# oiwn/toy-heaan-ckks

Measured on AMD Instinct MI355X. Metric: RNS-NTT poly-muls/sec (N=2^16, 16 primes) at 1/2/4/8 GPUs; % HBM roofline, higher is better.
Workload: dtype u32

## Files before the change

toy-heaan-ckks_amd/csrc/rnt_mfma.hip:

```cpp
#include <hip/hip_runtime.h>

#include <vector>

#include "rnt_internal.hpp"
#include "rnt_hostmath.hpp"
#include "rnt_modarith.hpp"
#include "rnt_device.hpp"

namespace rnt {

#ifdef RNT_MF_TRACE
constexpr int kMfTraceWg = 4096, kMfTraceSt = 16;
__device__ uint64_t g_mf_trace[kMfTraceWg * 16 * kMfTraceSt];
#define MF_STAMP(S)                                                                                  \
  do {                                                                                               \
    const uint32_t wg_ = blockIdx.x + blockIdx.y * gridDim.x;                                        \
    if ((threadIdx.x & 63u) == 0 && wg_ < (uint32_t)kMfTraceWg)                                      \
      g_mf_trace[(wg_ * 16 + (threadIdx.x >> 6)) * kMfTraceSt + (S)] = __builtin_amdgcn_s_memrealtime(); \
  } while (0)
#else
#define MF_STAMP(S) \
  do {              \
  } while (0)
#endif

namespace mf {

typedef int v4i __attribute__((ext_vector_type(4)));
constexpr int kT = 1024;
constexpr uint32_t kN = 1u << 16;
constexpr uint32_t K32 = 0x80808080u;

constexpr int S_F1 = 0, S_F2 = 1, S_F3 = 17, S_F4 = 18, S_I4 = 19, S_I3 = 20, S_I2 = 21, S_I1 = 37;
constexpr int kSlots = 38;
constexpr int kMat = 0;
constexpr int kCompF1 = kSlots * 4 * 64;
constexpr int kCompI4 = kCompF1 + 64;
constexpr int kTw3f = kCompI4 + 64;
constexpr int kTw4f = kTw3f + 1024;
constexpr int kTw4i = kTw4f + 16384;
constexpr int kTw3i = kTw4i + 16384;
constexpr int S_F4S = (kTw3i + 1024 + 255) / 256;
#ifndef RNT_MF_FOLD3
#define RNT_MF_FOLD3 1
#endif
#ifndef RNT_MF_FOLD4
#define RNT_MF_FOLD4 0
#endif
constexpr bool kFold3 = RNT_MF_FOLD3 != 0, kFold4 = RNT_MF_FOLD4 != 0;
constexpr int kFoldBase = (S_F4S + 1) * 256;
constexpr int kTwB3 = 1024, kTwB4 = 16384;
constexpr int kTw3fA = kFoldBase, kTw3iA = kTw3fA + 2 * kTwB3;
constexpr int kFold4Base = kFoldBase + (kFold3 ? 4 * kTwB3 : 0);
constexpr int kTw4fA = kFold4Base, kTw4iA = kTw4fA + 2 * kTwB4;
constexpr int kLimb = kFold4Base + (kFold4 ? 4 * kTwB4 : 0);
constexpr int kTw3iR = kFold3 ? kTw3iA : kTw3i;
constexpr int kTw4fR = kFold4 ? kTw4fA : kTw4f, kTw4iR = kFold4 ? kTw4iA : kTw4i;
constexpr bool kFold3Fwd = false;
constexpr size_t kLdsBytes = (size_t)160 * 1024;
static_assert(kLdsBytes > 80 * 1024, "one workgroup per CU");

__host__ __device__ constexpr int p3(int c, int i) {
  return 4 * (8 * (i >> 1) + 4 * (i & 1) + 2 * ((c >> 1) & 1) + (c & 1)) + 2 * (c >> 3) + ((c >> 2) & 1);
}
__host__ __device__ constexpr int q2(int c, int i) {
  return p3(8 * (i >> 1) + 4 * (i & 1) + 2 * (c >> 3) + ((c >> 2) & 1), 2 * ((c >> 1) & 1) + (c & 1));
}

struct Mc {
  int32_t q;
  uint32_t nqinv;
  int64_t K;
  int64_t K0;
  int32_t one;
  int32_t s16;
};

typedef __amdgpu_buffer_rsrc_t Rsrc;
__device__ __forceinline__ Rsrc rsrc(const void* base, uint32_t bytes) {
  return __builtin_amdgcn_make_buffer_rsrc((void*)base, 0, (int)bytes, 0x00020000);
}
#ifndef RNT_MF_NT
#define RNT_MF_NT 2
#endif
constexpr int kStreamAux = RNT_MF_NT;
#ifndef RNT_MF_LAST_NT
#define RNT_MF_LAST_NT 2
#endif
constexpr int kLastAux = RNT_MF_LAST_NT;
template <int AUX = 0>
__device__ __forceinline__ v4i bld(Rsrc r, uint32_t voff, uint32_t soff) {
  const auto v = __builtin_amdgcn_raw_buffer_load_b128(r, voff, soff, AUX);
  return v4i{(int)v[0], (int)v[1], (int)v[2], (int)v[3]};
}
template <int AUX = 0>
__device__ __forceinline__ void bst(v4i x, Rsrc r, uint32_t voff, uint32_t soff) {
  using V4 = decltype(__builtin_amdgcn_raw_buffer_load_b128(r, 0, 0, 0));
  V4 v;
  v[0] = (uint32_t)x[0];
  v[1] = (uint32_t)x[1];
  v[2] = (uint32_t)x[2];
  v[3] = (uint32_t)x[3];
  __builtin_amdgcn_raw_buffer_store_b128(v, r, voff, soff, AUX);
  asm volatile("s_nop 1" ::"v"(v));
}

template <bool WK>
__device__ __forceinline__ int32_t recomb(int32_t c0, int32_t c1, int32_t c2, int32_t c3, const Mc& m) {
  const int32_t lo = c0 + (int32_t)((uint32_t)c1 << 8);
  const int32_t hi = c2 + (int32_t)((uint32_t)c3 << 8);
  int64_t t;
  if constexpr (WK) {
    uint64_t cc;
    asm("v_mad_i64_i32 %0, %1, %2, 1, %3" : "=v"(t), "=s"(cc) : "v"(lo), "s"(m.K));
  } else {
    t = (int64_t)lo;
  }
  t = (int64_t)hi * m.s16 + t;
  const uint32_t mm = (uint32_t)t * m.nqinv;
  const int64_t v = (int64_t)(int32_t)mm * m.q + t;
  return (int32_t)(v >> 32);
}
template <bool WK>
__device__ __forceinline__ int32_t mont(int32_t a, int32_t b, const Mc& m) {
  int64_t p;
  uint64_t cc;
  asm("v_mad_i64_i32 %0, %1, %2, %3, %4" : "=v"(p), "=s"(cc) : "v"(a), "v"(b), "s"(WK ? m.K : m.K0));
  const uint32_t mm = (uint32_t)p * m.nqinv;
  const int64_t v = (int64_t)(int32_t)mm * m.q + p;
  return (int32_t)(v >> 32);
}
__device__ __forceinline__ int32_t recomb_tw(int32_t lo, int32_t hi, int32_t twA, int32_t twB, const Mc& m) {
  int64_t p0, p;
  uint64_t cc;
  asm("v_mad_i64_i32 %0, %1, %2, %3, %4" : "=v"(p0), "=s"(cc) : "v"(lo), "v"(twA), "s"(m.K));
  asm("v_mad_i64_i32 %0, %1, %2, %3, %4" : "=v"(p), "=s"(cc) : "v"(hi), "v"(twB), "v"(p0));
  const uint32_t mm = (uint32_t)p * m.nqinv;
  const int64_t v = (int64_t)(int32_t)mm * m.q + p;
  return (int32_t)(v >> 32);
}
template <bool LATE>
__device__ __forceinline__ void twist4(uint32_t (&o)[4], const v4i (&D)[4], v4i ta, Rsrc tab, uint32_t tvo,
                                       uint32_t tsa, uint32_t tsb, const Mc& m) {
  int32_t lo[4], hi[4];
#pragma unroll
  for (int i = 0; i < 4; ++i) {
    lo[i] = D[0][i] + (int32_t)((uint32_t)D[1][i] << 8);
    hi[i] = D[2][i] + (int32_t)((uint32_t)D[3][i] << 8);
  }
  __builtin_amdgcn_sched_barrier(0);
  if constexpr (LATE) ta = bld(tab, tvo, tsa);
  const v4i tb = bld(tab, tvo, tsb);
#pragma unroll
  for (int i = 0; i < 4; ++i) o[i] = (uint32_t)recomb_tw(lo[i], hi[i], ta[i], tb[i], m) ^ K32;
}
template <int DIST>
__device__ __forceinline__ uint32_t tw_b(uint32_t tso) {
  uint32_t v = tso + (uint32_t)DIST * 16u;
  asm volatile("" : "+s"(v));
  return v;
}
__device__ __forceinline__ void tile_fence() { __builtin_amdgcn_sched_barrier(0); }
__device__ __forceinline__ void pin4(uint32_t a, uint32_t b, uint32_t c, uint32_t d) {
  asm volatile("" ::"v"(a), "v"(b), "v"(c), "v"(d));
}
__device__ __forceinline__ uint32_t pk_canon(uint32_t x) { return (x + 0x40808080u) ^ K32; }
__device__ __forceinline__ uint32_t canon(int32_t r, int32_t q) { return (uint32_t)(r + ((r >> 31) & q)); }

template <bool DA, bool HC>
__device__ __forceinline__ void tile(v4i (&D)[4], const v4i (&M)[4], v4i dat, v4i c0) {
#define RNT_MF4(A0, B0, A1, B1, A2, B2, A3, B3, C0)                                  \
  "s_nop 1\n\t"                                                                      \
  "v_mfma_i32_16x16x64_i8 %0, " A0 ", " B0 ", " C0 "\n\t"                            \
  "v_mfma_i32_16x16x64_i8 %1, " A1 ", " B1 ", 0\n\t"                                 \
  "v_mfma_i32_16x16x64_i8 %2, " A2 ", " B2 ", 0\n\t"                                 \
  "v_mfma_i32_16x16x64_i8 %3, " A3 ", " B3 ", 0\n\t"                                 \
  "s_nop 7"
  if constexpr (DA && HC)
    asm volatile(RNT_MF4("%4", "%5", "%4", "%6", "%4", "%7", "%4", "%8", "%9")
                 : "=&v"(D[0]), "=&v"(D[1]), "=&v"(D[2]), "=&v"(D[3])
                 : "v"(dat), "v"(M[0]), "v"(M[1]), "v"(M[2]), "v"(M[3]), "v"(c0));
  else if constexpr (DA)
    asm volatile(RNT_MF4("%4", "%5", "%4", "%6", "%4", "%7", "%4", "%8", "0")
                 : "=&v"(D[0]), "=&v"(D[1]), "=&v"(D[2]), "=&v"(D[3])
                 : "v"(dat), "v"(M[0]), "v"(M[1]), "v"(M[2]), "v"(M[3]));
  else if constexpr (HC)
    asm volatile(RNT_MF4("%5", "%4", "%6", "%4", "%7", "%4", "%8", "%4", "%9")
                 : "=&v"(D[0]), "=&v"(D[1]), "=&v"(D[2]), "=&v"(D[3])
                 : "v"(dat), "v"(M[0]), "v"(M[1]), "v"(M[2]), "v"(M[3]), "v"(c0));
  else
    asm volatile(RNT_MF4("%5", "%4", "%6", "%4", "%7", "%4", "%8", "%4", "0")
                 : "=&v"(D[0]), "=&v"(D[1]), "=&v"(D[2]), "=&v"(D[3])
                 : "v"(dat), "v"(M[0]), "v"(M[1]), "v"(M[2]), "v"(M[3]));
#undef RNT_MF4
}
__device__ __forceinline__ void load_mat(v4i (&M)[4], Rsrc tab, uint32_t slot, uint32_t lo) {
#pragma unroll
  for (int a = 0; a < 4; ++a) M[a] = bld(tab, lo, (uint32_t)(kMat + (slot * 4 + a) * 64) * 16u);
}

struct Th {
  uint32_t tid0, w;
  __device__ explicit Th(uint32_t tt) : tid0(tt), w(__builtin_amdgcn_readfirstlane(tt >> 6)) {}
  __device__ __forceinline__ uint32_t t() const {
    uint32_t v = tid0;
    asm volatile("" : "+v"(v));
    return v;
  }
  __device__ __forceinline__ uint32_t lam() const { return t() & 63u; }
  __device__ __forceinline__ uint32_t g() const { return (t() >> 4) & 3u; }
  __device__ __forceinline__ uint32_t n() const { return t() & 15u; }
};

__device__ __forceinline__ void p1_bases(uint32_t (&wb)[4], const Th& h) {
  const uint32_t n0 = h.n() & 1, n1 = (h.n() >> 1) & 1, n2 = (h.n() >> 2) & 1, n3 = h.n() >> 3;
  const uint32_t g0 = h.g() & 1, g1 = h.g() >> 1;
  const uint32_t w0 = h.w & 1, w1 = (h.w >> 1) & 1, w2 = (h.w >> 2) & 1, w3 = h.w >> 3;
  const uint32_t rest = 4 * n0 + 8 * n1 + 16 * (w1 ^ g0) + 256 * w0 + 512 * w3 + 1024 * n2 + 2048 * n3 +
                        4096 * g0 + 8192 * g1 + 16384 * w2;
#pragma unroll
  for (uint32_t e = 0; e < 4; ++e) wb[e] = rest + ((e & 1) ^ n2) + 2 * ((e >> 1) ^ n3);
}
__device__ __forceinline__ void p2_bases(uint32_t (&rb)[4], const Th& h) {
  const uint32_t n0 = h.n() & 1, n1 = (h.n() >> 1) & 1, n2 = (h.n() >> 2) & 1, n3 = h.n() >> 3;
  const uint32_t g0 = h.g() & 1, g1 = h.g() >> 1;
  const uint32_t w0 = h.w & 1, w1 = (h.w >> 1) & 1, w2 = (h.w >> 2) & 1, w3 = h.w >> 3;
  const uint32_t rest = 4 * n2 + 8 * n3 + 16 * (g0 ^ w0) + 64 * w2 + 128 * w3 + 4096 * w0 + 8192 * w1 + 16384 * g1;
#pragma unroll
  for (uint32_t e = 0; e < 4; ++e) rb[e] = rest + (n0 ^ (e & 1)) + 2 * (n1 ^ (e >> 1)) + 1024 * (e & 1) + 2048 * (e >> 1);
}
__host__ __device__ constexpr uint32_t p1_off(int c, int i) { return 32u * ((c >> 2) & 1) + 64u * (i & 1) + 128u * (i >> 1); }
__host__ __device__ constexpr uint32_t p2_off(int c, int i) { return 32u * (i & 1) + 512u * (i >> 1) + 256u * ((c >> 2) & 1); }

template <uint32_t OFF>
__device__ __forceinline__ uint32_t lds_rd(uint32_t addr) {
  uint32_t v;
  asm volatile("ds_read_b32 %0, %1 offset:%2" : "=v"(v) : "v"(addr), "i"(OFF));
  return v;
}
template <int B0>
__device__ __forceinline__ void lds_wait8(uint32_t (&x)[64]) {
  asm volatile("s_waitcnt lgkmcnt(0)"
               : "+v"(x[B0 + 0]), "+v"(x[B0 + 1]), "+v"(x[B0 + 2]), "+v"(x[B0 + 3]), "+v"(x[B0 + 4]),
                 "+v"(x[B0 + 5]), "+v"(x[B0 + 6]), "+v"(x[B0 + 7]));
}

template <int H>
__device__ __forceinline__ void x_write_p1(const uint32_t (&x1)[64], uint32_t* lds, const uint32_t (&wb)[4]) {
#pragma unroll
  for (int c = 8 * H; c < 8 * H + 8; ++c)
#pragma unroll
    for (int i = 0; i < 4; ++i) lds[wb[c & 3] + p1_off(c, i)] = x1[4 * c + i];
}
template <int H, int C, int I>
__device__ __forceinline__ void x_read_p2_one(uint32_t (&x2)[64], uint32_t lds0, const uint32_t (&rb)[4]) {
  x2[4 * C + I] = lds_rd<p2_off(C, I) * 4u>(lds0 + rb[C & 3] * 4u);
}
template <int H>
__device__ __forceinline__ void x_read_p2(uint32_t (&x2)[64], const uint32_t* lds, const uint32_t (&rb)[4]) {
  const uint32_t l0 = (uint32_t)(uintptr_t)lds;
#define RNT_MF_RD(C)                      \
  x_read_p2_one<H, C, 0>(x2, l0, rb);     \
  x_read_p2_one<H, C, 1>(x2, l0, rb);     \
  x_read_p2_one<H, C, 2>(x2, l0, rb);     \
  x_read_p2_one<H, C, 3>(x2, l0, rb);
  RNT_MF_RD(8 * H + 0) RNT_MF_RD(8 * H + 1) RNT_MF_RD(8 * H + 2) RNT_MF_RD(8 * H + 3)
  RNT_MF_RD(8 * H + 4) RNT_MF_RD(8 * H + 5) RNT_MF_RD(8 * H + 6) RNT_MF_RD(8 * H + 7)
#undef RNT_MF_RD
  lds_wait8<32 * H + 0>(x2);
  lds_wait8<32 * H + 8>(x2);
  lds_wait8<32 * H + 16>(x2);
  lds_wait8<32 * H + 24>(x2);
}
__device__ __forceinline__ void p1_bases4(uint32_t (&wb)[4], const Th& h) {
  const uint32_t n0 = h.n() & 1, n1 = (h.n() >> 1) & 1, n2 = (h.n() >> 2) & 1, n3 = h.n() >> 3;
  const uint32_t g0 = h.g() & 1, g1 = h.g() >> 1;
  const uint32_t w0 = h.w & 1, w1 = (h.w >> 1) & 1, w2 = (h.w >> 2) & 1, w3 = h.w >> 3;
  const uint32_t rest = 4 * n0 + 8 * n1 + 16 * (w1 ^ g0) + 128 * w0 + 256 * w3 + 512 * n2 + 1024 * n3 +
                        2048 * g0 + 4096 * g1 + 8192 * w2;
#pragma unroll
  for (uint32_t e = 0; e < 4; ++e) wb[e] = rest + ((e & 1) ^ n2) + 2 * ((e >> 1) ^ n3);
}
__device__ __forceinline__ void p2_bases4(uint32_t (&rb)[4], const Th& h) {
  const uint32_t n0 = h.n() & 1, n1 = (h.n() >> 1) & 1, n2 = (h.n() >> 2) & 1, n3 = h.n() >> 3;
  const uint32_t g0 = h.g() & 1, g1 = h.g() >> 1;
  const uint32_t w0 = h.w & 1, w1 = (h.w >> 1) & 1, w2 = (h.w >> 2) & 1, w3 = h.w >> 3;
  const uint32_t rest = 4 * n2 + 8 * n3 + 16 * (g0 ^ w0) + 32 * w2 + 64 * w3 + 2048 * w0 + 4096 * w1 + 8192 * g1;
#pragma unroll
  for (uint32_t e = 0; e < 4; ++e) rb[e] = rest + (n0 ^ (e & 1)) + 2 * (n1 ^ (e >> 1)) + 512 * (e & 1) + 1024 * (e >> 1);
}
__host__ __device__ constexpr uint32_t p1_off4(int, int i) { return 32u * (i & 1) + 64u * (i >> 1); }
__host__ __device__ constexpr uint32_t p2_off4(int c, int i) { return 256u * (i >> 1) + 128u * ((c >> 2) & 1); }
template <int Q>
__device__ __forceinline__ void x_write_p1q(const uint32_t (&x1)[64], uint32_t* lds, const uint32_t (&wb)[4]) {
#pragma unroll
  for (int c = 4 * Q; c < 4 * Q + 4; ++c)
#pragma unroll
    for (int i = 0; i < 4; ++i) lds[wb[c & 3] + p1_off4(c, i)] = x1[4 * c + i];
}
template <int C, int I>
__device__ __forceinline__ void x_read_p2q_one(uint32_t (&x2)[64], uint32_t lds0, const uint32_t (&rb)[4]) {
  x2[4 * C + I] = lds_rd<p2_off4(C, I) * 4u>(lds0 + rb[C & 3] * 4u);
}
template <int Q>
__device__ __forceinline__ void x_read_p2q(uint32_t (&x2)[64], const uint32_t* lds, const uint32_t (&rb)[4]) {
  constexpr int H = Q >> 1, X = Q & 1;
  const uint32_t l0 = (uint32_t)(uintptr_t)lds;
#define RNT_MF_RDQ(C)                    \
  x_read_p2q_one<C, X>(x2, l0, rb);      \
  x_read_p2q_one<C, X + 2>(x2, l0, rb);
  RNT_MF_RDQ(8 * H + 0) RNT_MF_RDQ(8 * H + 1) RNT_MF_RDQ(8 * H + 2) RNT_MF_RDQ(8 * H + 3)
  RNT_MF_RDQ(8 * H + 4) RNT_MF_RDQ(8 * H + 5) RNT_MF_RDQ(8 * H + 6) RNT_MF_RDQ(8 * H + 7)
#undef RNT_MF_RDQ
  constexpr int B = 32 * H + X;
  asm volatile("s_waitcnt lgkmcnt(0)"
               : "+v"(x2[B + 0]), "+v"(x2[B + 2]), "+v"(x2[B + 4]), "+v"(x2[B + 6]), "+v"(x2[B + 8]),
                 "+v"(x2[B + 10]), "+v"(x2[B + 12]), "+v"(x2[B + 14]), "+v"(x2[B + 16]), "+v"(x2[B + 18]),
                 "+v"(x2[B + 20]), "+v"(x2[B + 22]), "+v"(x2[B + 24]), "+v"(x2[B + 26]), "+v"(x2[B + 28]),
                 "+v"(x2[B + 30]));
}
template <int H>
__device__ __forceinline__ void x_write_p2(const uint32_t (&x2)[64], uint32_t* lds, const uint32_t (&rb)[4]) {
#pragma unroll
  for (int c = 8 * H; c < 8 * H + 8; ++c)
#pragma unroll
    for (int i = 0; i < 4; ++i) lds[rb[c & 3] + p2_off(c, i)] = x2[q2(c, i)];
}
template <int H, int C, int I>
__device__ __forceinline__ void x_read_p1_one(uint32_t (&x1)[64], uint32_t lds0, const uint32_t (&wb)[4]) {
  x1[4 * C + I] = lds_rd<p1_off(C, I) * 4u>(lds0 + wb[C & 3] * 4u);
}
template <int H>
__device__ __forceinline__ void x_read_p1(uint32_t (&x1)[64], const uint32_t* lds, const uint32_t (&wb)[4]) {
  const uint32_t l0 = (uint32_t)(uintptr_t)lds;
#define RNT_MF_RD(C)                      \
  x_read_p1_one<H, C, 0>(x1, l0, wb);     \
  x_read_p1_one<H, C, 1>(x1, l0, wb);     \
  x_read_p1_one<H, C, 2>(x1, l0, wb);     \
  x_read_p1_one<H, C, 3>(x1, l0, wb);
  RNT_MF_RD(8 * H + 0) RNT_MF_RD(8 * H + 1) RNT_MF_RD(8 * H + 2) RNT_MF_RD(8 * H + 3)
  RNT_MF_RD(8 * H + 4) RNT_MF_RD(8 * H + 5) RNT_MF_RD(8 * H + 6) RNT_MF_RD(8 * H + 7)
#undef RNT_MF_RD
  lds_wait8<32 * H + 0>(x1);
  lds_wait8<32 * H + 8>(x1);
  lds_wait8<32 * H + 16>(x1);
  lds_wait8<32 * H + 24>(x1);
}

__device__ __forceinline__ void swap_p2p3(uint32_t (&x)[64]) {
#pragma unroll
  for (int c = 0; c < 16; ++c) {
    if (c & 2) continue;
#pragma unroll
    for (int i = 0; i < 4; ++i) {
      const auto r = __builtin_amdgcn_permlane32_swap(x[4 * c + i], x[4 * (c | 2) + i], false, false);
      x[4 * c + i] = r[0];
      x[4 * (c | 2) + i] = r[1];
    }
  }
#pragma unroll
  for (int c = 0; c < 16; ++c) {
    if (c & 1) continue;
#pragma unroll
    for (int i = 0; i < 4; ++i) {
      const auto r = __builtin_amdgcn_permlane16_swap(x[4 * c + i], x[4 * (c | 1) + i], false, false);
      x[4 * c + i] = r[0];
      x[4 * (c | 1) + i] = r[1];
    }
  }
}
__device__ __forceinline__ void swap_q3p2(uint32_t (&x)[64]) {
#pragma unroll
  for (int c = 0; c < 16; ++c) {
    if (c & 2) continue;
#pragma unroll
    for (int i = 0; i < 4; ++i) {
      const auto r = __builtin_amdgcn_permlane32_swap(x[p3(c, i)], x[p3(c | 2, i)], false, false);
      x[p3(c, i)] = r[0];
      x[p3(c | 2, i)] = r[1];
    }
  }
#pragma unroll
  for (int c = 0; c < 16; ++c) {
    if (c & 1) continue;
#pragma unroll
    for (int i = 0; i < 4; ++i) {
      const auto r = __builtin_amdgcn_permlane16_swap(x[p3(c, i)], x[p3(c | 1, i)], false, false);
      x[p3(c, i)] = r[0];
      x[p3(c | 1, i)] = r[1];
    }
  }
}

#ifndef RNT_MF_PRIO
#define RNT_MF_PRIO 1
#endif
#ifndef RNT_MF_TENSOR_SYNCX
#define RNT_MF_TENSOR_SYNCX 1
#endif
#ifndef RNT_MF_TENSOR_PARK
#define RNT_MF_TENSOR_PARK 0
#endif
#ifndef RNT_MF_TENSOR_MEAS
#define RNT_MF_TENSOR_MEAS 0
#endif
#ifndef RNT_MF_TENSOR_PARK4
#define RNT_MF_TENSOR_PARK4 0
#endif
#ifndef RNT_MF_IPRIO
#define RNT_MF_IPRIO 1
#endif
#ifndef RNT_MF_PRIO_VAR
#define RNT_MF_PRIO_VAR 0
#endif
template <bool ON>
__device__ __forceinline__ void mf_prio(int p) {
  if constexpr (ON) {
    constexpr int s1 = RNT_MF_PRIO_VAR ? 20 : 10, s2 = RNT_MF_PRIO_VAR ? 28 : 20, s3 = RNT_MF_PRIO_VAR ? 34 : 30;
    if (p == 0) __builtin_amdgcn_s_setprio(3);
    if (p == s1) __builtin_amdgcn_s_setprio(2);
    if (p == s2) __builtin_amdgcn_s_setprio(1);
    if (p == s3) __builtin_amdgcn_s_setprio(0);
  }
}
template <int C0, bool BIAS>
__device__ __forceinline__ void pass_p1(uint32_t (&x1)[64], const v4i (&M)[4], v4i comp, const Mc& m) {
#pragma unroll
  for (int c = C0; c < C0 + 8; ++c) {
    v4i b;
#pragma unroll
    for (int i = 0; i < 4; ++i) b[i] = (int)(BIAS ? pk_canon(x1[4 * c + i]) : x1[4 * c + i]);
    v4i D[4];
    tile<false, BIAS>(D, M, b, comp);
#pragma unroll
    for (int i = 0; i < 4; ++i) x1[4 * c + i] = (uint32_t)recomb<true>(D[0][i], D[1][i], D[2][i], D[3][i], m) ^ K32;
    pin4(x1[4 * c + 0], x1[4 * c + 1], x1[4 * c + 2], x1[4 * c + 3]);
    tile_fence();
  }
}
template <int C0, bool FOLD>
__device__ __forceinline__ void pass_p2(uint32_t (&x2)[64], const v4i (&M)[4], Rsrc tab, uint32_t tvo, uint32_t tso,
                                        const Mc& m) {
  const uint32_t tsb = FOLD ? tw_b<kTwB3>(tso) : tso;
  const v4i z = {0, 0, 0, 0};
#pragma unroll
  for (int c = C0; c < C0 + 8; ++c) {
    if constexpr (C0 == 8) mf_prio<RNT_MF_PRIO != 0>(c - 8);
    v4i b;
#pragma unroll
    for (int i = 0; i < 4; ++i) b[i] = (int)x2[4 * c + i];
    const v4i tv = FOLD ? z : bld(tab, tvo, tso + (uint32_t)c * 16u);
    v4i D[4];
    tile<false, false>(D, M, b, z);
    if constexpr (FOLD) {
      uint32_t o[4];
      twist4<true>(o, D, tv, tab, tvo, tso + (uint32_t)c * 16u, tsb + (uint32_t)c * 16u, m);
#pragma unroll
      for (int i = 0; i < 4; ++i) x2[4 * c + i] = o[i];
    } else {
#pragma unroll
      for (int i = 0; i < 4; ++i) {
        const int32_t r = recomb<false>(D[0][i], D[1][i], D[2][i], D[3][i], m);
        x2[4 * c + i] = (uint32_t)mont<true>(r, tv[i], m) ^ K32;
      }
    }
    pin4(x2[4 * c + 0], x2[4 * c + 1], x2[4 * c + 2], x2[4 * c + 3]);
    tile_fence();
  }
}
__device__ __forceinline__ void pass_p3(uint32_t (&x)[64], const v4i (&M)[4], Rsrc tab, uint32_t tvo, uint32_t tso,
                                        const Mc& m) {
  const uint32_t tsb = kFold4 ? tw_b<kTwB4>(tso) : tso;
  const v4i z = {0, 0, 0, 0};
#pragma unroll
  for (int c = 0; c < 16; ++c) {
    mf_prio<RNT_MF_PRIO != 0>(8 + c);
    v4i a;
#pragma unroll
    for (int i = 0; i < 4; ++i) a[i] = (int)x[p3(c, i)];
    const v4i tv = bld(tab, tvo, tso + (uint32_t)c * 1024u);
    v4i D[4];
    tile<true, false>(D, M, a, z);
    if constexpr (kFold4) {
      uint32_t o[4];
      twist4<false>(o, D, tv, tab, tvo, 0, tsb + (uint32_t)c * 1024u, m);
#pragma unroll
      for (int i = 0; i < 4; ++i) x[p3(c, i)] = o[i];
    } else {
#pragma unroll
      for (int i = 0; i < 4; ++i) {
        const int32_t r = recomb<false>(D[0][i], D[1][i], D[2][i], D[3][i], m);
        x[p3(c, i)] = (uint32_t)mont<true>(r, tv[i], m) ^ K32;
      }
    }
    pin4(x[p3(c, 0)], x[p3(c, 1)], x[p3(c, 2)], x[p3(c, 3)]);
    tile_fence();
  }
}
template <class EPI>
__device__ __forceinline__ void pass_p4(uint32_t (&x)[64], const v4i (&M)[4], const Mc& m, const EPI& epi) {
  const v4i z = {0, 0, 0, 0};
#pragma unroll
  for (int c = 0; c < 16; ++c) {
    mf_prio<RNT_MF_PRIO != 0>(24 + c);
    v4i b;
#pragma unroll
    for (int i = 0; i < 4; ++i) b[i] = (int)x[p3(c, i)];
    v4i D[4];
    tile<false, false>(D, M, b, z);
    int32_t r[4];
#pragma unroll
    for (int i = 0; i < 4; ++i) r[i] = recomb<false>(D[0][i], D[1][i], D[2][i], D[3][i], m);
    epi(c, r, x);
    tile_fence();
  }
}
constexpr int kStash = 10;
static_assert((size_t)kStash * 16 * 1024 <= kLdsBytes, "sixteen waves' stashes in the LDS");
__device__ __forceinline__ uint32_t stash_addr(const uint32_t* lds, const Th& h) {
  return (uint32_t)(uintptr_t)lds + (h.w * (kStash * 64u) + h.lam()) * 16u;
}
__device__ __forceinline__ void stash_put(uint32_t addr, int c, uint32_t a, uint32_t b, uint32_t d, uint32_t e) {
  asm volatile("ds_write_b128 %0, %1 offset:%2" ::"v"(addr), "v"(v4i{(int)a, (int)b, (int)d, (int)e}), "i"(c * 1024)
               : "memory");
}
__device__ __forceinline__ v4i stash_get(uint32_t addr, int c) {
  v4i v;
  asm volatile("ds_read_b128 %0, %1 offset:%2\n\ts_waitcnt lgkmcnt(0)" : "=v"(v) : "v"(addr), "i"(c * 1024) : "memory");
  return v;
}
template <bool PK = false>
__device__ __forceinline__ void ipass_p4(uint32_t (&x)[64], const v4i (&M)[4], v4i comp, v4i tv, Rsrc tab,
                                         uint32_t tvo, uint32_t tso, const Mc& m, uint32_t* lds, const Th& h) {
  const uint32_t tsb = kFold4 ? tw_b<kTwB4>(tso) : tso;
#pragma unroll
  for (int c = 0; c < 16; ++c) {
    mf_prio<RNT_MF_IPRIO != 0>(c);
    v4i a;
#pragma unroll
    for (int i = 0; i < 4; ++i) a[i] = (int)(PK ? x[p3(c, i)] : pk_canon(x[p3(c, i)]));
    const v4i tn = c + 1 < 16 ? bld(tab, tvo, tso + (uint32_t)(c + 1) * 1024u) : tv;
    v4i D[4];
    if constexpr (PK)
      tile<true, false>(D, M, a, v4i{0, 0, 0, 0});
    else
      tile<true, true>(D, M, a, comp);
    if constexpr (kFold4) {
      uint32_t o[4];
      twist4<false>(o, D, tv, tab, tvo, 0, tsb + (uint32_t)c * 1024u, m);
#pragma unroll
      for (int i = 0; i < 4; ++i) x[p3(c, i)] = o[i];
    } else {
#pragma unroll
      for (int i = 0; i < 4; ++i) {
        const int32_t r = recomb<false>(D[0][i], D[1][i], D[2][i], D[3][i], m);
        x[p3(c, i)] = (uint32_t)mont<true>(r, tv[i], m) ^ K32;
      }
    }
    if (c < kStash)
      stash_put(stash_addr(lds, h), c, x[p3(c, 0)], x[p3(c, 1)], x[p3(c, 2)], x[p3(c, 3)]);
    else
      pin4(x[p3(c, 0)], x[p3(c, 1)], x[p3(c, 2)], x[p3(c, 3)]);
    tv = tn;
    tile_fence();
  }
}
__device__ __forceinline__ void ipass_p3(uint32_t (&x)[64], const v4i (&M)[4], Rsrc tab, uint32_t tvo, uint32_t tso,
                                         const Mc& m, uint32_t* lds, const Th& h) {
  const uint32_t tsb = kFold3 ? tw_b<kTwB3>(tso) : tso;
  const v4i z = {0, 0, 0, 0};
#pragma unroll
  for (int c = 0; c < 16; ++c) {
    mf_prio<RNT_MF_IPRIO != 0>(16 + c);
    v4i b;
    if (c < kStash) {
      b = stash_get(stash_addr(lds, h), c);
    } else {
#pragma unroll
      for (int i = 0; i < 4; ++i) b[i] = (int)x[p3(c, i)];
    }
    const v4i tv = kFold3 ? z : bld(tab, tvo, tso + (uint32_t)c * 64u);
    v4i D[4];
    tile<false, false>(D, M, b, z);
    if constexpr (kFold3) {
      uint32_t o[4];
      twist4<true>(o, D, tv, tab, tvo, tso + (uint32_t)c * 64u, tsb + (uint32_t)c * 64u, m);
#pragma unroll
      for (int i = 0; i < 4; ++i) x[p3(c, i)] = o[i];
    } else {
#pragma unroll
      for (int i = 0; i < 4; ++i) {
        const int32_t r = recomb<false>(D[0][i], D[1][i], D[2][i], D[3][i], m);
        x[p3(c, i)] = (uint32_t)mont<true>(r, tv[i], m) ^ K32;
      }
    }
    pin4(x[p3(c, 0)], x[p3(c, 1)], x[p3(c, 2)], x[p3(c, 3)]);
    tile_fence();
  }
}
template <int C0>
__device__ __forceinline__ void ipass_p2(uint32_t (&x)[64], const v4i (&M)[4], const Mc& m) {
  const v4i z = {0, 0, 0, 0};
#pragma unroll
  for (int c = C0; c < C0 + 8; ++c) {
    if constexpr (C0 == 0) mf_prio<RNT_MF_IPRIO != 0>(32 + c);
    v4i b;
#pragma unroll
    for (int i = 0; i < 4; ++i) b[i] = (int)x[q2(c, i)];
    v4i D[4];
    tile<false, false>(D, M, b, z);
#pragma unroll
    for (int i = 0; i < 4; ++i)
      x[q2(c, i)] = (uint32_t)recomb<true>(D[0][i], D[1][i], D[2][i], D[3][i], m) ^ K32;
    pin4(x[q2(c, 0)], x[q2(c, 1)], x[q2(c, 2)], x[q2(c, 3)]);
    tile_fence();
  }
}
template <int C0>
__device__ __forceinline__ void ipass_p1(uint32_t (&x1)[64], const v4i (&M)[4], const Mc& m, Rsrc dst,
                                         const Th& h);

__device__ __forceinline__ uint32_t p1_lane(const Th& h) { return ((h.g() << 12) | (h.n() << 2)) * 4u; }
__device__ __forceinline__ uint32_t p1_wave(const Th& h) {
  const uint32_t w = h.w;
  return (((w >> 3) << 11) | (((w >> 2) & 1) << 9) | (((w >> 1) & 1) << 8) | ((w & 1) << 6)) * 4u;
}
__host__ __device__ constexpr uint32_t p1_reg(int i, int hc) {
  return (((uint32_t)i << 14) | ((uint32_t)(hc & 1) << 10) | ((uint32_t)(hc >> 1) << 7)) * 4u;
}
__device__ __forceinline__ void load_p1(uint32_t (&x1)[64], Rsrc src, const Th& h) {
  const uint32_t lo = p1_lane(h), wo = p1_wave(h);
#pragma unroll
  for (int hc = 0; hc < 4; ++hc)
#pragma unroll
    for (int i = 0; i < 4; ++i) {
      const v4i v = bld<kStreamAux>(src, lo, wo + p1_reg(i, hc));
#pragma unroll
      for (int e = 0; e < 4; ++e) x1[4 * (4 * hc + e) + i] = (uint32_t)v[e];
    }
}
template <int C0>
__device__ __forceinline__ void ipass_p1(uint32_t (&x1)[64], const v4i (&M)[4], const Mc& m, Rsrc dst,
                                         const Th& h) {
  const v4i z = {0, 0, 0, 0};
#pragma unroll
  for (int c = C0; c < C0 + 8; ++c) {
    v4i b;
#pragma unroll
    for (int i = 0; i < 4; ++i) b[i] = (int)x1[4 * c + i];
    v4i D[4];
    tile<false, false>(D, M, b, z);
#pragma unroll
    for (int i = 0; i < 4; ++i) x1[4 * c + i] = canon(recomb<false>(D[0][i], D[1][i], D[2][i], D[3][i], m), m.q);
    if ((c & 3) == 3) {
      const int hc = c >> 2;
      const uint32_t lo = p1_lane(h), wo = p1_wave(h);
#pragma unroll
      for (int i = 0; i < 4; ++i) {
        v4i v;
#pragma unroll
        for (int e = 0; e < 4; ++e) v[e] = (int)x1[4 * (4 * hc + e) + i];
        bst<kStreamAux>(v, dst, lo, wo + p1_reg(i, hc));
      }
    } else {
      pin4(x1[4 * c + 0], x1[4 * c + 1], x1[4 * c + 2], x1[4 * c + 3]);
    }
    tile_fence();
  }
}

__device__ __forceinline__ uint32_t p4_lane(const Th& h) { return ((h.n() << 4) | (h.g() << 2)) * 4u; }
__device__ __forceinline__ uint32_t p4_soff(const Th& h, int c) { return ((h.w << 12) | ((uint32_t)c << 8)) * 4u; }

struct Tabs {
  Rsrc tab;
  Mc m;
};
__device__ __forceinline__ Tabs tabs_of(const void* mf, const LimbConst<uint32_t>& lc, uint32_t l) {
  Tabs r;
  r.tab = rsrc((const v4i*)mf + (size_t)l * kLimb, (uint32_t)kLimb * 16u);
  r.m.q = (int32_t)lc.q;
  r.m.nqinv = 0u - lc.qinv;
  int64_t K = (int64_t)((uint64_t)K32 << 32), K0 = 0;
  int32_t one = 1, s16 = 65536;
  asm volatile("" : "+s"(one), "+s"(s16), "+s"(K), "+s"(K0));
  r.m.K = K;
  r.m.K0 = K0;
  r.m.one = one;
  r.m.s16 = s16;
  return r;
}

struct NoEpi {
  __device__ void operator()(int, const int32_t (&)[4], uint32_t (&)[64]) const {}
};
template <int NPARK, uint32_t PBASE, uint32_t PSTRIDE>
__device__ __forceinline__ uint32_t park_addr(const uint32_t* lds, const Th& h) {
  static_assert(NPARK * 1024 <= (int)PSTRIDE && PBASE + 16 * PSTRIDE <= kLdsBytes, "park area");
  return (uint32_t)(uintptr_t)lds + PBASE + h.w * PSTRIDE + h.lam() * 16u;
}
template <bool SYNC1, int F4 = S_F4, bool Q4 = false, bool SYNCX = false, int NPARK = 0, uint32_t PBASE = 0,
          uint32_t PSTRIDE = 0, bool F3 = kFold3, class EPI = NoEpi>
__device__ __forceinline__ void fwd(uint32_t (&x2)[64], Rsrc src, uint32_t* lds, const Th& h, const Tabs& T,
                                    const EPI& epi = EPI{}) {
  const Mc& m = T.m;
  const uint32_t lo = h.lam() * 16u;
  v4i M[4];
  load_mat(M, T.tab, S_F1, lo);
  const v4i comp = bld(T.tab, lo, (uint32_t)kCompF1 * 16u);
  uint32_t x1[64];
  load_p1(x1, src, h);
  MF_STAMP(1);
  pass_p1<0, true>(x1, M, comp, m);
  MF_STAMP(2);
  if constexpr (SYNC1) __syncthreads();
  uint32_t wb[4], rb[4];
  const uint32_t t3v = h.g() * 256u, t3s = (uint32_t)((F3 ? kTw3fA : kTw3f) + h.w * 64) * 16u;
  if constexpr (Q4) {
    p1_bases4(wb, h);
    x_write_p1q<0>(x1, lds, wb);
    pass_p1<8, true>(x1, M, comp, m);
    __syncthreads();
    p2_bases4(rb, h);
    x_read_p2q<0>(x2, lds, rb);
    __syncthreads();
    p1_bases4(wb, h);
    x_write_p1q<1>(x1, lds, wb);
    __syncthreads();
    p2_bases4(rb, h);
    x_read_p2q<1>(x2, lds, rb);
    __syncthreads();
    p1_bases4(wb, h);
    x_write_p1q<2>(x1, lds, wb);
    load_mat(M, T.tab, S_F2 + h.w, lo);
    pass_p2<0, F3>(x2, M, T.tab, t3v, t3s, m);
    __syncthreads();
    p2_bases4(rb, h);
    x_read_p2q<2>(x2, lds, rb);
    __syncthreads();
    p1_bases4(wb, h);
    x_write_p1q<3>(x1, lds, wb);
    __syncthreads();
    p2_bases4(rb, h);
    x_read_p2q<3>(x2, lds, rb);
  } else {
  p1_bases(wb, h);
  x_write_p1<0>(x1, lds, wb);
  pass_p1<8, true>(x1, M, comp, m);
  MF_STAMP(3);
  __syncthreads();
  MF_STAMP(4);
  p2_bases(rb, h);
  x_read_p2<0>(x2, lds, rb);
  __syncthreads();
  MF_STAMP(5);
  p1_bases(wb, h);
  x_write_p1<1>(x1, lds, wb);
  load_mat(M, T.tab, S_F2 + h.w, lo);
  pass_p2<0, F3>(x2, M, T.tab, t3v, t3s, m);
  MF_STAMP(6);
  __syncthreads();
  MF_STAMP(7);
  p2_bases(rb, h);
  x_read_p2<1>(x2, lds, rb);
  }
  if constexpr (SYNCX) __syncthreads();
  static_assert(NPARK == 0 || SYNCX, "the park area is free only past SYNCX");
#pragma unroll
  for (int c = 0; c < NPARK; ++c)
    stash_put(park_addr<NPARK, PBASE, PSTRIDE>(lds, h), c, x2[4 * c], x2[4 * c + 1], x2[4 * c + 2], x2[4 * c + 3]);
  pass_p2<8, F3>(x2, M, T.tab, t3v, t3s, m);
  MF_STAMP(8);
#pragma unroll
  for (int c = 0; c < NPARK; ++c) {
    const v4i v = stash_get(park_addr<NPARK, PBASE, PSTRIDE>(lds, h), c);
#pragma unroll
    for (int i = 0; i < 4; ++i) x2[4 * c + i] = (uint32_t)v[i];
  }
  swap_p2p3(x2);
  load_mat(M, T.tab, S_F3, lo);
  pass_p3(x2, M, T.tab, lo, (uint32_t)(kTw4fR + h.w * 1024) * 16u, m);
  MF_STAMP(9);
  load_mat(M, T.tab, F4, lo);
  pass_p4(x2, M, m, epi);
  MF_STAMP(10);
}

template <bool LOAD, bool PK = false>
__device__ __forceinline__ void inv_x(uint32_t (&x2)[64], Rsrc pr, uint32_t* lds, const Th& h, const Tabs& T) {
  const Mc& m = T.m;
  const uint32_t lo = h.lam() * 16u;
  v4i M[4];
  load_mat(M, T.tab, S_I4, lo);
  const v4i comp = bld(T.tab, lo, (uint32_t)kCompI4 * 16u);
  const uint32_t t4s = (uint32_t)(kTw4iR + h.w * 1024) * 16u;
  const v4i tv0 = bld(T.tab, lo, t4s);
  if constexpr (LOAD) {
#pragma unroll
    for (int cc = 0; cc < 16; ++cc) {
      const v4i v = bld<kStreamAux>(pr, p4_lane(h), p4_soff(h, cc));
#pragma unroll
      for (int i = 0; i < 4; ++i) x2[p3(cc, i)] = (uint32_t)v[i];
    }
  } else {
    __syncthreads();
  }
  ipass_p4<PK>(x2, M, comp, tv0, T.tab, lo, t4s, m, lds, h);
  load_mat(M, T.tab, S_I3, lo);
  ipass_p3(x2, M, T.tab, h.g() * 16u, (uint32_t)(kTw3iR + h.w * 64) * 16u, m, lds, h);
  swap_q3p2(x2);
  load_mat(M, T.tab, S_I2 + h.w, lo);
  uint32_t wb[4], rb[4];
  uint32_t x1[64];
  ipass_p2<0>(x2, M, m);
  __syncthreads();
  p2_bases(rb, h);
  x_write_p2<0>(x2, lds, rb);
  ipass_p2<8>(x2, M, m);
  __syncthreads();
  p1_bases(wb, h);
  x_read_p1<0>(x1, lds, wb);
  __syncthreads();
  p2_bases(rb, h);
  x_write_p2<1>(x2, lds, rb);
  load_mat(M, T.tab, S_I1, lo);
  ipass_p1<0>(x1, M, m, pr, h);
  __syncthreads();
  p1_bases(wb, h);
  x_read_p1<1>(x1, lds, wb);
  ipass_p1<8>(x1, M, m, pr, h);
}
__device__ __forceinline__ void inv(Rsrc pr, uint32_t* lds, const Th& h, const Tabs& T) {
  uint32_t x2[64];
  inv_x<true>(x2, pr, lds, h, T);
}

}

template <bool INV>
__global__ void __launch_bounds__(mf::kT, 1)
k_mf_ntt(uint32_t* __restrict__ data, const void* __restrict__ mft, const LimbConst<uint32_t>* __restrict__ lcs,
         uint64_t ls) {
  using namespace mf;
  extern __shared__ __attribute__((aligned(16))) unsigned char smem_raw[];
  uint32_t* lds = (uint32_t*)smem_raw;
  const Th h(threadIdx.x);
  const uint32_t poly = blockIdx.x, l = blockIdx.y;
  MF_STAMP(0);
  uint32_t* p = data + (uint64_t)l * ls + (uint64_t)poly * kN;
  const Tabs T = tabs_of(mft, lcs[l], l);
  const Rsrc pr = rsrc(p, kN * 4u);
  if constexpr (!INV) {
    uint32_t x[64];
    fwd<false, S_F4, false, false, 0, 0, 0, kFold3 && kFold3Fwd>(x, pr, lds, h, T, [&](int cc, const int32_t (&r)[4], uint32_t (&)[64]) {
      bst<kStreamAux>(v4i{(int)canon(r[0], T.m.q), (int)canon(r[1], T.m.q), (int)canon(r[2], T.m.q), (int)canon(r[3], T.m.q)}, pr,
          p4_lane(h), p4_soff(h, cc));
    });
  } else {
    inv(pr, lds, h, T);
  }
#ifdef RNT_MF_TRACE
  __builtin_amdgcn_s_waitcnt(0);
  MF_STAMP(11);
#endif
}

__global__ void __launch_bounds__(mf::kT, 1)
k_mf_tensor(uint32_t* __restrict__ d0, uint32_t* __restrict__ d1, uint32_t* __restrict__ d2, uint64_t ols,
            const uint32_t* __restrict__ c0, const uint32_t* __restrict__ c1, const uint32_t* __restrict__ c0p,
            const uint32_t* __restrict__ c1p, uint64_t ils, uint32_t* __restrict__ scratch, uint32_t slots,
            const void* __restrict__ mft, const LimbConst<uint32_t>* __restrict__ lcs,
            uint32_t* __restrict__ d2hat) {
  using namespace mf;
  extern __shared__ __attribute__((aligned(16))) unsigned char smem_raw[];
  uint32_t* lds = (uint32_t*)smem_raw;
  const Th h(threadIdx.x);
  const uint32_t poly = blockIdx.x, l = blockIdx.y;
  const uint64_t oo = (uint64_t)l * ols + (uint64_t)poly * kN, io = (uint64_t)l * ils + (uint64_t)poly * kN;
  const LimbConst<uint32_t> lc = lcs[l];
  const Tabs T = tabs_of(mft, lc, l);
  const uint32_t q = lc.q, nqi = T.m.nqinv;
  uint64_t so;
  if (slots) {
    const uint32_t xcc = __builtin_amdgcn_s_getreg((31 << 11) | 20) & 7u;
    const uint32_t cu = (__builtin_amdgcn_s_getreg((31 << 11) | 4) >> 8) & 0xffu;
    so = (uint64_t)((xcc << 8) | cu) << 16;
  } else {
    so = (uint64_t)(poly + l * gridDim.x) << 16;
  }
  const Rsrc R0 = rsrc(d0 + oo, kN * 4u), R1 = rsrc(d1 + oo, kN * 4u), R2 = rsrc(d2 + oo, kN * 4u);
  const Rsrc RS = rsrc(scratch + so, kN * 4u);
  const bool want_hat = d2hat != nullptr;
  const Rsrc RH = rsrc(want_hat ? d2hat + oo : d2 + oo, kN * 4u);
  const uint32_t pl = p4_lane(h);
  auto canon4 = [q](const int32_t (&r)[4]) {
    return v4i{(int)canon(r[0], (int32_t)q), (int)canon(r[1], (int32_t)q), (int)canon(r[2], (int32_t)q),
               (int)canon(r[3], (int32_t)q)};
  };
  auto mmul = [q, nqi](uint32_t a, uint32_t b) {
    const uint64_t t = (uint64_t)a * b;
    const uint32_t mm = (uint32_t)t * nqi;
    const uint32_t r = (uint32_t)((t + (uint64_t)mm * q) >> 32);
    return r >= q ? r - q : r;
  };
  const uint32_t rm = lc.rmod, rmp = lc.rmod_p;
  uint32_t x[64];
  constexpr bool SX = RNT_MF_TENSOR_SYNCX != 0;
  constexpr int NP = SX ? RNT_MF_TENSOR_PARK : 0;
  constexpr uint32_t PB = 128u * 1024u, PS = 2048u;
  constexpr int MEAS = RNT_MF_TENSOR_MEAS;
  fwd<false, S_F4, false, SX, NP, PB, PS>(x, rsrc(c0 + io, kN * 4u), lds, h, T, [&](int cc, const int32_t (&r)[4], uint32_t (&)[64]) {
    if constexpr (MEAS != 3) bst(canon4(r), R1, pl, p4_soff(h, cc));
  });
  fwd<!SX, S_F4, false, SX, NP, PB, PS>(x, rsrc(c1 + io, kN * 4u), lds, h, T, [&](int cc, const int32_t (&r)[4], uint32_t (&)[64]) {
    if constexpr (MEAS != 1) bst(canon4(r), RS, pl, p4_soff(h, cc));
  });
  fwd<!SX, S_F4, false, SX, NP, PB, PS>(x, rsrc(c0p + io, kN * 4u), lds, h, T, [&](int cc, const int32_t (&r)[4], uint32_t (&)[64]) {
    const v4i a0 = MEAS == 3 ? canon4(r) : bld(R1, pl, p4_soff(h, cc));
    const v4i a1 = MEAS == 1 ? canon4(r) : bld(RS, pl, p4_soff(h, cc));
    const v4i b = canon4(r);
    v4i o0, t;
#pragma unroll
    for (int i = 0; i < 4; ++i) {
      o0[i] = (int)mmul((uint32_t)a0[i], (uint32_t)b[i]);
      t[i] = (int)mmul((uint32_t)a1[i], (uint32_t)b[i]);
    }
    bst<kLastAux>(o0, R0, pl, p4_soff(h, cc));
    if constexpr (MEAS != 2) bst(t, R2, pl, p4_soff(h, cc));
  });
  fwd<!SX, S_F4, false, RNT_MF_TENSOR_PARK4 && SX, RNT_MF_TENSOR_PARK4 ? NP : 0, PB, PS>(x, rsrc(c1p + io, kN * 4u), lds, h, T, [&](int cc, const int32_t (&r)[4], uint32_t (&xx)[64]) {
    const v4i b = canon4(r);
    const v4i a0 = MEAS == 3 ? b : bld<kLastAux>(R1, pl, p4_soff(h, cc));
    const v4i a1 = MEAS == 1 ? b : bld<kLastAux>(RS, pl, p4_soff(h, cc));
    const v4i t = MEAS == 2 ? b : bld<kLastAux>(R2, pl, p4_soff(h, cc));
    v4i o1;
#pragma unroll
    for (int i = 0; i < 4; ++i) {
      const uint32_t s = (uint32_t)t[i] + mmul((uint32_t)a0[i], (uint32_t)b[i]);
      o1[i] = (int)(s >= q ? s - q : s);
      const uint32_t m = mmul((uint32_t)a1[i], (uint32_t)b[i]);
      const uint32_t qh = (uint32_t)(((uint64_t)m * rmp) >> 32);
      const uint32_t v = m * rm - qh * q;
      xx[p3(cc, i)] = v >= q ? v - q : v;
    }
    pin4(xx[p3(cc, 0)], xx[p3(cc, 1)], xx[p3(cc, 2)], xx[p3(cc, 3)]);
    bst<kLastAux>(o1, R1, pl, p4_soff(h, cc));
    if (want_hat)
      bst<kLastAux>(v4i{(int)xx[p3(cc, 0)], (int)xx[p3(cc, 1)], (int)xx[p3(cc, 2)], (int)xx[p3(cc, 3)]}, RH, pl,
                    p4_soff(h, cc));
  });
  inv_x<false>(x, R2, lds, h, T);
}

#ifndef RNT_MF_MUL_Q4
#define RNT_MF_MUL_Q4 1
#endif
#ifndef RNT_MF_MUL_NOSYNC1
#define RNT_MF_MUL_NOSYNC1 1
#endif
#ifndef RNT_MF_MUL_PARK
#define RNT_MF_MUL_PARK 4
#endif
#ifndef RNT_MF_MUL_MEAS
#define RNT_MF_MUL_MEAS 0
#endif
#ifndef RNT_MF_SLOT_ST_AUX
#define RNT_MF_SLOT_ST_AUX 0
#endif
#ifndef RNT_MF_MUL_MEAS_SKIP
#define RNT_MF_MUL_MEAS_SKIP (RNT_MF_MUL_MEAS ? 16 - kMulLdsTiles : 0)
#endif
constexpr int kMulLdsTiles = RNT_MF_MUL_Q4 ? 6 : 2;
constexpr uint32_t kMulLdsBase = RNT_MF_MUL_Q4 ? (1u << 14) : (1u << 15);
static_assert(kMulLdsBase * 4 + (size_t)kMulLdsTiles * 16 * 1024 <= mf::kLdsBytes, "in the LDS");
__global__ void __launch_bounds__(mf::kT, 1)
k_mf_mul(uint32_t* c, const uint32_t* a, const uint32_t* b, uint64_t ls, uint32_t* __restrict__ scratch,
         uint32_t slots, const void* __restrict__ mft, const LimbConst<uint32_t>* __restrict__ lcs) {
  using namespace mf;
  extern __shared__ __attribute__((aligned(16))) unsigned char smem_raw[];
  uint32_t* lds = (uint32_t*)smem_raw;
  const Th h(threadIdx.x);
  const uint32_t poly = blockIdx.x, l = blockIdx.y;
  const uint64_t o = (uint64_t)l * ls + (uint64_t)poly * kN;
  const LimbConst<uint32_t> lc = lcs[l];
  const Tabs T = tabs_of(mft, lc, l);
  uint64_t so;
  if (slots) {
    const uint32_t xcc = __builtin_amdgcn_s_getreg((31 << 11) | 20) & 7u;
    const uint32_t cu = (__builtin_amdgcn_s_getreg((31 << 11) | 4) >> 8) & 0xffu;
    so = (uint64_t)((xcc << 8) | cu) << 16;
  } else {
    so = (uint64_t)(poly + l * gridDim.x) << 16;
  }
  const Rsrc RS = rsrc(scratch + so, kN * 4u);
  uint32_t x[64];
  auto hat = [&](int t) -> v4i& { return ((v4i*)(lds + kMulLdsBase) + h.w * (kMulLdsTiles * 64) + h.lam())[t * 64]; };
  constexpr int NP = RNT_MF_MUL_Q4 ? RNT_MF_MUL_PARK : 0;
  fwd<false, S_F4S, false, RNT_MF_MUL_Q4 != 0, NP, kMulLdsBase * 4, kMulLdsTiles * 1024>(x, rsrc(a + o, kN * 4u), lds, h, T, [&](int cc, const int32_t (&r)[4], uint32_t (&)[64]) {
    if (cc >= 16 - kMulLdsTiles)
      hat(cc - (16 - kMulLdsTiles)) = v4i{r[0], r[1], r[2], r[3]};
    else if (cc >= RNT_MF_MUL_MEAS_SKIP)
      bst<RNT_MF_SLOT_ST_AUX>(v4i{r[0], r[1], r[2], r[3]}, RS, p4_lane(h), p4_soff(h, cc));
  });
  fwd<!(RNT_MF_MUL_Q4 && RNT_MF_MUL_NOSYNC1), S_F4, RNT_MF_MUL_Q4 != 0, (NP > 0), NP, 0, 4096>(x, rsrc(b + o, kN * 4u), lds, h, T, [&](int cc, const int32_t (&r)[4], uint32_t (&xx)[64]) {
    const v4i ah = cc >= 16 - kMulLdsTiles ? hat(cc - (16 - kMulLdsTiles))
                   : cc < RNT_MF_MUL_MEAS_SKIP ? v4i{r[0], r[1], r[2], r[3]} : bld(RS, p4_lane(h), p4_soff(h, cc));
#pragma unroll
    for (int i = 0; i < 4; ++i) {
      xx[p3(cc, i)] = (uint32_t)mont<true>(ah[i], r[i], T.m) ^ K32;
    }
    pin4(xx[p3(cc, 0)], xx[p3(cc, 1)], xx[p3(cc, 2)], xx[p3(cc, 3)]);
  });
  inv_x<false, true>(x, rsrc(c + o, kN * 4u), lds, h, T);
}

namespace {
using host::brv;
using host::invmod;
using host::mulmod;
using host::powmod;

int32_t centred(uint64_t v, uint64_t q) {
  v %= q;
  return v > q / 2 ? (int32_t)((int64_t)v - (int64_t)q) : (int32_t)v;
}

void expand(const uint64_t (&W)[16][16], uint64_t q, uint64_t R, bool DA, int KAP, int32_t* out) {
  int32_t E[16][16][4];
  for (int o = 0; o < 16; ++o)
    for (int k = 0; k < 16; ++k)
      for (int b = 0; b < 4; ++b) E[o][k][b] = centred(mulmod(mulmod(W[o][k], (1ull << (8 * b)) % q, q), R, q), q);
  for (int a = 0; a < 4; ++a)
    for (int lam = 0; lam < 64; ++lam)
      for (int i = 0; i < 4; ++i) {
        const int g = lam >> 4, r = lam & 15;
        const int kin = KAP ? 4 * g + i : 4 * i + g;
        const int jout = DA ? r : (KAP ? r : 4 * (r & 3) + (r >> 2));
        uint32_t wd = 0;
        for (int b = 0; b < 4; ++b) {
          const uint32_t u = (uint32_t)E[jout][kin][b] + 0x80808080u;
          wd |= ((((u >> (8 * a)) & 0xFFu) ^ 0x80u) & 0xFFu) << (8 * b);
        }
        out[(a * 64 + lam) * 4 + i] = (int32_t)wd;
      }
}

}

int mf_build(Tables* t, std::string* err) {
  using namespace mf;
  const size_t L = t->L;
  const uint64_t n = kN;
  std::vector<int32_t> all((size_t)L * kLimb * 4);
  std::vector<uint64_t> tw(n), itw(n), pw(n), ipw(n);
  for (size_t l = 0; l < L; ++l) {
    const uint64_t q = t->moduli[l], psi = t->psi[l], psinv = invmod(psi, q);
    uint64_t x = 1, y = 1;
    for (uint64_t j = 0; j < n; ++j) {
      pw[j] = x;
      ipw[j] = y;
      x = mulmod(x, psi, q);
      y = mulmod(y, psinv, q);
    }
    for (uint64_t g = 0; g < n; ++g) {
      tw[g] = pw[brv(g, 16)];
      itw[g] = ipw[brv(g, 16)];
    }
    const uint64_t R = (uint64_t)(((host::u128)1 << 32) % q);
    {
      const double rb = (double)q / 2 + 16384.0;
      if (rb * rb / 4294967296.0 + (double)q / 2 + 1 >= (double)0x7F7F7F7Fu) {
        *err = "MFMA tables: the product bound exceeds the packed digit range for this prime";
        return -1;
      }
      if ((kFold3 || kFold4) &&
          (268435456.0 + 1048576.0) * (double)q / 4294967296.0 + (double)q / 2 + 1 >= (double)0x7F7F7F7Fu) {
        *err = "MFMA tables: the folded twist bound exceeds the packed digit range for this prime";
        return -1;
      }
    }
    uint64_t M0[16][16];
    for (int k = 0; k < 16; ++k) {
      uint64_t v[16] = {};
      v[k] = 1;
      for (int sb = 3; sb >= 0; --sb) {
        const int b = 12 + sb;
        for (int kk = 0; kk < 16; ++kk) {
          if (kk & (1 << sb)) continue;
          const uint64_t i = (uint64_t)kk << 12;
          const uint64_t w = tw[(n + i) >> (b + 1)];
          const uint64_t x = v[kk], y = v[kk | (1 << sb)];
          const uint64_t tt = mulmod(w, y, q);
          v[kk] = (x + tt) % q;
          v[kk | (1 << sb)] = (x + q - tt) % q;
        }
      }
      for (int j = 0; j < 16; ++j) M0[j][k] = v[j];
    }
    const uint64_t beta1i = itw[8];
    uint64_t F[16][16], Fi[16][16];
    const uint64_t inv16 = invmod(16 % q, q);
    for (int j = 0; j < 16; ++j)
      for (int k = 0; k < 16; ++k) F[j][k] = mulmod(M0[j][k], powmod(beta1i, (uint64_t)k, q), q);
    for (int j = 0; j < 16; ++j)
      for (int k = 0; k < 16; ++k) Fi[k][j] = mulmod(inv16, invmod(F[j][k], q), q);
    for (int j = 0; j < 16; ++j)
      for (int k = 0; k < 16; ++k) {
        uint64_t s = 0;
        for (int x = 0; x < 16; ++x) s = (s + mulmod(F[j][x], Fi[x][k], q)) % q;
        if (s != (j == k ? 1u : 0u)) {
          *err = "MFMA tables: F is not invertible as a DFT";
          return -1;
        }
      }
    int32_t* lt = all.data() + l * (size_t)kLimb * 4;
    auto slot = [&](int s) { return lt + (size_t)(kMat + s * 4 * 64) * 4; };
    uint64_t W[16][16];
    expand(M0, q, R, false, 0, slot(S_F1));
    for (int U = 0; U < 16; ++U) {
      const uint64_t be = tw[128 + 8 * U], bei = itw[128 + 8 * U];
      for (int j = 0; j < 16; ++j)
        for (int k = 0; k < 16; ++k) W[j][k] = mulmod(F[j][k], powmod(be, (uint64_t)k, q), q);
      expand(W, q, R, false, 0, slot(S_F2 + U));
      for (int k = 0; k < 16; ++k)
        for (int j = 0; j < 16; ++j) W[k][j] = mulmod(powmod(bei, (uint64_t)k, q), Fi[k][j], q);
      expand(W, q, R, false, 0, slot(S_I2 + U));
    }
    expand(F, q, R, true, 0, slot(S_F3));
    expand(F, q, R, false, 1, slot(S_F4));
    for (int j = 0; j < 16; ++j)
      for (int k = 0; k < 16; ++k) W[j][k] = mulmod(F[j][k], R, q);
    expand(W, q, R, false, 1, slot(S_F4S));
    expand(Fi, q, R, true, 1, slot(S_I4));
    expand(Fi, q, R, false, 1, slot(S_I3));
    for (int k = 0; k < 16; ++k)
      for (int j = 0; j < 16; ++j) W[k][j] = mulmod(powmod(beta1i, (uint64_t)k, q), Fi[k][j], q);
    expand(W, q, R, false, 0, slot(S_I1));
    const uint64_t bias = mulmod(R, (1ull << 30) % q, q);
    {
      int32_t cf[16], ci[16];
      for (int j = 0; j < 16; ++j) {
        uint64_t s0 = 0, s1 = 0;
        for (int k = 0; k < 16; ++k) {
          s0 = (s0 + M0[j][k]) % q;
          s1 = (s1 + Fi[j][k]) % q;
        }
        cf[j] = centred(mulmod(bias, s0, q), q);
        ci[j] = centred(mulmod(bias, s1, q), q);
      }
      int32_t* c1 = lt + (size_t)kCompF1 * 4;
      int32_t* c4 = lt + (size_t)kCompI4 * 4;
      for (int lam = 0; lam < 64; ++lam)
        for (int i = 0; i < 4; ++i) {
          c1[lam * 4 + i] = cf[4 * i + (lam >> 4)];
          c4[lam * 4 + i] = ci[lam & 15];
        }
    }
    const uint64_t s16 = (1ull << 16) % q;
    auto put = [&](int32_t* tab, bool fold, int dist, size_t idx, uint64_t tv) {
      if (fold) {
        tab[idx] = centred(tv, q);
        tab[(size_t)dist * 4 + idx] = centred(mulmod(tv, s16, q), q);
      } else {
        tab[idx] = centred(mulmod(tv, R, q), q);
      }
    };
    int32_t* t3f = lt + (size_t)kTw3f * 4;
    int32_t* t3fa = lt + (size_t)kTw3fA * 4;
    int32_t* t3i = lt + (size_t)kTw3iR * 4;
    for (int w = 0; w < 16; ++w)
      for (int g = 0; g < 4; ++g)
        for (int c = 0; c < 16; ++c)
          for (int i = 0; i < 4; ++i) {
            const int U3 = (w << 4) | (i << 2) | g;
            const uint64_t tv = powmod(tw[2048 + 8 * U3], (uint64_t)c, q);
            put(t3f, false, 0, ((w * 4 + g) * 16 + c) * 4 + i, tv);
            if (kFold3) put(t3fa, true, kTwB3, ((w * 4 + g) * 16 + c) * 4 + i, tv);
          }
    for (int w = 0; w < 16; ++w)
      for (int c = 0; c < 16; ++c)
        for (int g = 0; g < 4; ++g)
          for (int i = 0; i < 4; ++i) {
            const int U3 = (w << 4) | c;
            put(t3i, kFold3, kTwB3, ((w * 16 + c) * 4 + g) * 4 + i, powmod(itw[2048 + 8 * U3], (uint64_t)(4 * g + i), q));
          }
    int32_t* t4f = lt + (size_t)kTw4fR * 4;
    int32_t* t4i = lt + (size_t)kTw4iR * 4;
    for (int w = 0; w < 16; ++w)
      for (int c = 0; c < 16; ++c)
        for (int lam = 0; lam < 64; ++lam)
          for (int i = 0; i < 4; ++i) {
            const int g = lam >> 4, nn = lam & 15;
            const int Uf = (w << 8) | (c << 4) | nn;
            put(t4f, kFold4, kTwB4, ((w * 16 + c) * 64 + lam) * 4 + i, powmod(tw[32768 + 8 * Uf], (uint64_t)(4 * g + i), q));
            const int Ui = (w << 8) | (c << 4) | (4 * g + i);
            put(t4i, kFold4, kTwB4, ((w * 16 + c) * 64 + lam) * 4 + i, powmod(itw[32768 + 8 * Ui], (uint64_t)nn, q));
          }
  }
  const size_t bytes = all.size() * sizeof(int32_t);
  void* dev = nullptr;
  if (hipError_t e = hipMalloc(&dev, bytes); e != hipSuccess) {
    *err = std::string("hipMalloc(MFMA tables): ") + hipGetErrorString(e);
    return -3;
  }
  if (hipError_t e = hipMemcpy(dev, all.data(), bytes, hipMemcpyHostToDevice); e != hipSuccess) {
    (void)hipFree(dev);
    *err = std::string("hipMemcpy(MFMA tables): ") + hipGetErrorString(e);
    return -2;
  }
  t->mf = dev;
  return 0;
}

static hipError_t launch_ntt_t(const Launch& k, const void* fn, void* data, uint64_t ls) {
  hipError_t e = hipFuncSetAttribute(fn, hipFuncAttributeMaxDynamicSharedMemorySize, (int)mf::kLdsBytes);
  if (e != hipSuccess) return e;
  uint32_t* d = (uint32_t*)data;
  const void* mft = (const mf::v4i*)k.t->mf + (size_t)k.tab0 * mf::kLimb;
  const LimbConst<uint32_t>* lcs = (const LimbConst<uint32_t>*)k.t->lconst + k.tab0;
  void* args[] = {&d, &mft, &lcs, &ls};
  return hipLaunchKernel(fn, dim3((unsigned)k.B, (unsigned)k.L), dim3(mf::kT), args, mf::kLdsBytes, k.s);
}

hipError_t launch_mf_tensor(const Launch& k, void* d0, void* d1, void* d2, uint64_t ols, const void* c0,
                            const void* c1, const void* c0p, const void* c1p, uint64_t ils, void* scratch) {
  if (k.B == 0 || k.L == 0) return hipSuccess;
  if (k.B > 0x7fffffffull || k.L > 65535) return hipErrorInvalidConfiguration;
  const void* fn = (const void*)k_mf_tensor;
  hipError_t e = hipFuncSetAttribute(fn, hipFuncAttributeMaxDynamicSharedMemorySize, (int)mf::kLdsBytes);
  if (e != hipSuccess) return e;
  uint32_t slots = (uint64_t)k.B * k.L >= kPlaneSlots ? 1u : 0u;
  const void* mft = k.t->mf;
  const LimbConst<uint32_t>* lcs = (const LimbConst<uint32_t>*)k.t->lconst;
  void* d2hat = k.d2hat;
  void* args[] = {&d0, &d1, &d2, &ols, &c0, &c1, &c0p, &c1p, &ils, &scratch, &slots, &mft, &lcs, &d2hat};
  return hipLaunchKernel(fn, dim3((unsigned)k.B, (unsigned)k.L), dim3(mf::kT), args, mf::kLdsBytes, k.s);
}

hipError_t launch_mf_mul(const Launch& k, void* c, const void* a, const void* b, uint64_t ls, void* scratch) {
  if (k.B == 0 || k.L == 0) return hipSuccess;
  if (k.B > 0x7fffffffull || k.L > 65535) return hipErrorInvalidConfiguration;
  const void* fn = (const void*)k_mf_mul;
  hipError_t e = hipFuncSetAttribute(fn, hipFuncAttributeMaxDynamicSharedMemorySize, (int)mf::kLdsBytes);
  if (e != hipSuccess) return e;
  uint32_t slots = (uint64_t)k.B * k.L >= kPlaneSlots ? 1u : 0u;
  const void* mft = k.t->mf;
  const LimbConst<uint32_t>* lcs = (const LimbConst<uint32_t>*)k.t->lconst;
  void* args[] = {&c, &a, &b, &ls, &scratch, &slots, &mft, &lcs};
  return hipLaunchKernel(fn, dim3((unsigned)k.B, (unsigned)k.L), dim3(mf::kT), args, mf::kLdsBytes, k.s);
}

#ifdef RNT_MF_TRACE
extern "C" __attribute__((visibility("default"))) int rnt_debug_mf_trace(uint64_t* out) {
  return (int)hipMemcpyFromSymbol(out, HIP_SYMBOL(g_mf_trace), sizeof(g_mf_trace));
}
#endif

hipError_t launch_mf_ntt(const Launch& k, int inverse, void* data, uint64_t ls) {
  if (k.B == 0 || k.L == 0) return hipSuccess;
  if (k.B > 0x7fffffffull || k.L > 65535) return hipErrorInvalidConfiguration;
  return inverse ? launch_ntt_t(k, (const void*)k_mf_ntt<true>, data, ls)
                 : launch_ntt_t(k, (const void*)k_mf_ntt<false>, data, ls);
}

}
```

Baseline: 165,700.

## Replace Montgomery recombination with Barrett-style quotient-estimate reduction in MFMA passes

Adds a second reduction scheme for the MFMA-based NTT passes. The digit partial sums are recombined into a 32-bit value and reduced with a mulhi-based quotient estimate (mu = 2^48/q) instead of a 64-bit Montgomery multiply-reduce. It builds plain (non-Montgomery-scaled) matrix tables and split bias constants, and injects an offset constant through the MFMA accumulator inputs. It is on by default for multiply, inverse NTT, tensor paths and the first forward pass, aiming to cut per-element VALU work. In exchange it uses extra table space per limb and tighter bounds checks that some primes may fail.

```diff
diff --git a/toy-heaan-ckks_amd/csrc/rnt_mfma.hip b/toy-heaan-ckks_amd/csrc/rnt_mfma.hip
--- a/toy-heaan-ckks_amd/csrc/rnt_mfma.hip
+++ b/toy-heaan-ckks_amd/csrc/rnt_mfma.hip
@@ -53,7 +53,35 @@
 constexpr int kTw3fA = kFoldBase, kTw3iA = kTw3fA + 2 * kTwB3;
 constexpr int kFold4Base = kFoldBase + (kFold3 ? 4 * kTwB3 : 0);
 constexpr int kTw4fA = kFold4Base, kTw4iA = kTw4fA + 2 * kTwB4;
-constexpr int kLimb = kFold4Base + (kFold4 ? 4 * kTwB4 : 0);
+#ifndef RNT_MF_QR
+#define RNT_MF_QR 3
+#endif
+#ifndef RNT_MF_QR_MUL
+#define RNT_MF_QR_MUL RNT_MF_QR
+#endif
+#ifndef RNT_MF_QR_NTT
+#define RNT_MF_QR_NTT RNT_MF_QR
+#endif
+#ifndef RNT_MF_QR_NTTF
+#define RNT_MF_QR_NTTF (RNT_MF_QR & 1)
+#endif
+#ifndef RNT_MF_QR_TENSOR
+#define RNT_MF_QR_TENSOR RNT_MF_QR
+#endif
+constexpr int kQrMul = RNT_MF_QR_MUL & 3, kQrNtt = RNT_MF_QR_NTT & 3, kQrNttFwd = RNT_MF_QR_NTTF & 3;
+constexpr int kQrTensor = RNT_MF_QR_TENSOR & 3;
+constexpr bool kQrAny = (kQrMul | kQrNtt | kQrNttFwd | kQrTensor) != 0;
+constexpr int kQrP4 = 4;
+constexpr int kQrBase = kFold4Base + (kFold4 ? 4 * kTwB4 : 0);
+static_assert(kQrBase % 256 == 0, "matrix slots are 256 v4i");
+constexpr int S_QF1 = kQrBase / 256, S_QF3 = S_QF1 + 1, S_QF4 = S_QF1 + 2, S_QI4 = S_QF1 + 3, S_QI2 = S_QF1 + 4;
+constexpr int kQCompF1 = (S_QI2 + 16) * 256, kQCompI4 = kQCompF1 + 128;
+constexpr int kQConst = kQCompI4 + 128;
+constexpr int kQrEnd = kQConst + 64;
+constexpr int kLimb = kQrAny ? kQrEnd : kQrBase;
+static_assert(!kQrAny || (kQConst < kLimb && (S_QI2 + 16) * 256 <= kQCompF1), "the plain slots lie inside the limb's table");
+#define RNT_MF_QRC "48"
+constexpr uint32_t kQrC = 48;
 constexpr int kTw3iR = kFold3 ? kTw3iA : kTw3i;
 constexpr int kTw4fR = kFold4 ? kTw4fA : kTw4f, kTw4iR = kFold4 ? kTw4iA : kTw4i;
 constexpr bool kFold3Fwd = false;
@@ -74,6 +102,8 @@
   int64_t K0;
   int32_t one;
   int32_t s16;
+  int32_t mu;
+  uint32_t nq, kq, kq0;
 };
 
 typedef __amdgpu_buffer_rsrc_t Rsrc;
@@ -122,6 +152,23 @@
   return (int32_t)(v >> 32);
 }
 template <bool WK>
+__device__ __forceinline__ int32_t recomb_q(int32_t c0, int32_t c1, int32_t c2, int32_t c3, const Mc& m) {
+  uint32_t lo = (uint32_t)c0 + ((uint32_t)c1 << 8);
+  uint32_t hi = (uint32_t)c2 + ((uint32_t)c3 << 8);
+  asm("" : "+v"(lo), "+v"(hi));
+  uint32_t t = (hi << 16) + lo;
+  asm("" : "+v"(t));
+  const int32_t qt = __mulhi((int32_t)hi, m.mu);
+  return (int32_t)(t + (uint32_t)qt * m.nq + (WK ? m.kq : m.kq0));
+}
+template <bool QR, bool WK>
+__device__ __forceinline__ int32_t recomb_x(int32_t c0, int32_t c1, int32_t c2, int32_t c3, const Mc& m) {
+  if constexpr (QR)
+    return recomb_q<WK>(c0, c1, c2, c3, m);
+  else
+    return recomb<WK>(c0, c1, c2, c3, m);
+}
+template <bool WK>
 __device__ __forceinline__ int32_t mont(int32_t a, int32_t b, const Mc& m) {
   int64_t p;
   uint64_t cc;
@@ -167,29 +214,45 @@
 __device__ __forceinline__ uint32_t pk_canon(uint32_t x) { return (x + 0x40808080u) ^ K32; }
 __device__ __forceinline__ uint32_t canon(int32_t r, int32_t q) { return (uint32_t)(r + ((r >> 31) & q)); }
 
-template <bool DA, bool HC>
-__device__ __forceinline__ void tile(v4i (&D)[4], const v4i (&M)[4], v4i dat, v4i c0) {
-#define RNT_MF4(A0, B0, A1, B1, A2, B2, A3, B3, C0)                                  \
+template <bool DA, bool HC, bool QC = false>
+__device__ __forceinline__ void tile(v4i (&D)[4], const v4i (&M)[4], v4i dat, v4i c0, v4i c2 = v4i{0, 0, 0, 0}) {
+#define RNT_MF4(A0, B0, A1, B1, A2, B2, A3, B3, C0, C2, C3)                          \
   "s_nop 1\n\t"                                                                      \
   "v_mfma_i32_16x16x64_i8 %0, " A0 ", " B0 ", " C0 "\n\t"                            \
   "v_mfma_i32_16x16x64_i8 %1, " A1 ", " B1 ", 0\n\t"                                 \
-  "v_mfma_i32_16x16x64_i8 %2, " A2 ", " B2 ", 0\n\t"                                 \
-  "v_mfma_i32_16x16x64_i8 %3, " A3 ", " B3 ", 0\n\t"                                 \
+  "v_mfma_i32_16x16x64_i8 %2, " A2 ", " B2 ", " C2 "\n\t"                            \
+  "v_mfma_i32_16x16x64_i8 %3, " A3 ", " B3 ", " C3 "\n\t"                            \
   "s_nop 7"
-  if constexpr (DA && HC)
-    asm volatile(RNT_MF4("%4", "%5", "%4", "%6", "%4", "%7", "%4", "%8", "%9")
+  if constexpr (QC && DA && HC)
+    asm volatile(RNT_MF4("%4", "%5", "%4", "%6", "%4", "%7", "%4", "%8", "%9", "%10", RNT_MF_QRC)
+                 : "=&v"(D[0]), "=&v"(D[1]), "=&v"(D[2]), "=&v"(D[3])
+                 : "v"(dat), "v"(M[0]), "v"(M[1]), "v"(M[2]), "v"(M[3]), "v"(c0), "v"(c2));
+  else if constexpr (QC && DA)
+    asm volatile(RNT_MF4("%4", "%5", "%4", "%6", "%4", "%7", "%4", "%8", "0", "0", RNT_MF_QRC)
+                 : "=&v"(D[0]), "=&v"(D[1]), "=&v"(D[2]), "=&v"(D[3])
+                 : "v"(dat), "v"(M[0]), "v"(M[1]), "v"(M[2]), "v"(M[3]));
+  else if constexpr (QC && HC)
+    asm volatile(RNT_MF4("%5", "%4", "%6", "%4", "%7", "%4", "%8", "%4", "%9", "%10", RNT_MF_QRC)
+                 : "=&v"(D[0]), "=&v"(D[1]), "=&v"(D[2]), "=&v"(D[3])
+                 : "v"(dat), "v"(M[0]), "v"(M[1]), "v"(M[2]), "v"(M[3]), "v"(c0), "v"(c2));
+  else if constexpr (QC)
+    asm volatile(RNT_MF4("%5", "%4", "%6", "%4", "%7", "%4", "%8", "%4", "0", "0", RNT_MF_QRC)
+                 : "=&v"(D[0]), "=&v"(D[1]), "=&v"(D[2]), "=&v"(D[3])
+                 : "v"(dat), "v"(M[0]), "v"(M[1]), "v"(M[2]), "v"(M[3]));
+  else if constexpr (DA && HC)
+    asm volatile(RNT_MF4("%4", "%5", "%4", "%6", "%4", "%7", "%4", "%8", "%9", "0", "0")
                  : "=&v"(D[0]), "=&v"(D[1]), "=&v"(D[2]), "=&v"(D[3])
                  : "v"(dat), "v"(M[0]), "v"(M[1]), "v"(M[2]), "v"(M[3]), "v"(c0));
   else if constexpr (DA)
-    asm volatile(RNT_MF4("%4", "%5", "%4", "%6", "%4", "%7", "%4", "%8", "0")
+    asm volatile(RNT_MF4("%4", "%5", "%4", "%6", "%4", "%7", "%4", "%8", "0", "0", "0")
                  : "=&v"(D[0]), "=&v"(D[1]), "=&v"(D[2]), "=&v"(D[3])
                  : "v"(dat), "v"(M[0]), "v"(M[1]), "v"(M[2]), "v"(M[3]));
   else if constexpr (HC)
-    asm volatile(RNT_MF4("%5", "%4", "%6", "%4", "%7", "%4", "%8", "%4", "%9")
+    asm volatile(RNT_MF4("%5", "%4", "%6", "%4", "%7", "%4", "%8", "%4", "%9", "0", "0")
                  : "=&v"(D[0]), "=&v"(D[1]), "=&v"(D[2]), "=&v"(D[3])
                  : "v"(dat), "v"(M[0]), "v"(M[1]), "v"(M[2]), "v"(M[3]), "v"(c0));
   else
-    asm volatile(RNT_MF4("%5", "%4", "%6", "%4", "%7", "%4", "%8", "%4", "0")
+    asm volatile(RNT_MF4("%5", "%4", "%6", "%4", "%7", "%4", "%8", "%4", "0", "0", "0")
                  : "=&v"(D[0]), "=&v"(D[1]), "=&v"(D[2]), "=&v"(D[3])
                  : "v"(dat), "v"(M[0]), "v"(M[1]), "v"(M[2]), "v"(M[3]));
 #undef RNT_MF4
@@ -423,17 +486,17 @@
     if (p == s3) __builtin_amdgcn_s_setprio(0);
   }
 }
-template <int C0, bool BIAS>
-__device__ __forceinline__ void pass_p1(uint32_t (&x1)[64], const v4i (&M)[4], v4i comp, const Mc& m) {
+template <int C0, bool BIAS, bool QR = false>
+__device__ __forceinline__ void pass_p1(uint32_t (&x1)[64], const v4i (&M)[4], v4i comp, v4i comp2, const Mc& m) {
 #pragma unroll
   for (int c = C0; c < C0 + 8; ++c) {
     v4i b;
 #pragma unroll
     for (int i = 0; i < 4; ++i) b[i] = (int)(BIAS ? pk_canon(x1[4 * c + i]) : x1[4 * c + i]);
     v4i D[4];
-    tile<false, BIAS>(D, M, b, comp);
-#pragma unroll
-    for (int i = 0; i < 4; ++i) x1[4 * c + i] = (uint32_t)recomb<true>(D[0][i], D[1][i], D[2][i], D[3][i], m) ^ K32;
+    tile<false, BIAS, QR>(D, M, b, comp, comp2);
+#pragma unroll
+    for (int i = 0; i < 4; ++i) x1[4 * c + i] = (uint32_t)recomb_x<QR, true>(D[0][i], D[1][i], D[2][i], D[3][i], m) ^ K32;
     pin4(x1[4 * c + 0], x1[4 * c + 1], x1[4 * c + 2], x1[4 * c + 3]);
     tile_fence();
   }
@@ -468,8 +531,10 @@
     tile_fence();
   }
 }
+template <bool QR = false>
 __device__ __forceinline__ void pass_p3(uint32_t (&x)[64], const v4i (&M)[4], Rsrc tab, uint32_t tvo, uint32_t tso,
                                         const Mc& m) {
+  static_assert(!(QR && kFold4), "a folded pass keeps the Montgomery matrix");
   const uint32_t tsb = kFold4 ? tw_b<kTwB4>(tso) : tso;
   const v4i z = {0, 0, 0, 0};
 #pragma unroll
@@ -480,7 +545,7 @@
     for (int i = 0; i < 4; ++i) a[i] = (int)x[p3(c, i)];
     const v4i tv = bld(tab, tvo, tso + (uint32_t)c * 1024u);
     v4i D[4];
-    tile<true, false>(D, M, a, z);
+    tile<true, false, QR>(D, M, a, z);
     if constexpr (kFold4) {
       uint32_t o[4];
       twist4<false>(o, D, tv, tab, tvo, 0, tsb + (uint32_t)c * 1024u, m);
@@ -489,7 +554,7 @@
     } else {
 #pragma unroll
       for (int i = 0; i < 4; ++i) {
-        const int32_t r = recomb<false>(D[0][i], D[1][i], D[2][i], D[3][i], m);
+        const int32_t r = recomb_x<QR, false>(D[0][i], D[1][i], D[2][i], D[3][i], m);
         x[p3(c, i)] = (uint32_t)mont<true>(r, tv[i], m) ^ K32;
       }
     }
@@ -497,7 +562,7 @@
     tile_fence();
   }
 }
-template <class EPI>
+template <bool QR = false, class EPI>
 __device__ __forceinline__ void pass_p4(uint32_t (&x)[64], const v4i (&M)[4], const Mc& m, const EPI& epi) {
   const v4i z = {0, 0, 0, 0};
 #pragma unroll
@@ -507,10 +572,10 @@
 #pragma unroll
     for (int i = 0; i < 4; ++i) b[i] = (int)x[p3(c, i)];
     v4i D[4];
-    tile<false, false>(D, M, b, z);
+    tile<false, false, QR>(D, M, b, z);
     int32_t r[4];
 #pragma unroll
-    for (int i = 0; i < 4; ++i) r[i] = recomb<false>(D[0][i], D[1][i], D[2][i], D[3][i], m);
+    for (int i = 0; i < 4; ++i) r[i] = recomb_x<QR, false>(D[0][i], D[1][i], D[2][i], D[3][i], m);
     epi(c, r, x);
     tile_fence();
   }
@@ -529,9 +594,10 @@
   asm volatile("ds_read_b128 %0, %1 offset:%2\n\ts_waitcnt lgkmcnt(0)" : "=v"(v) : "v"(addr), "i"(c * 1024) : "memory");
   return v;
 }
-template <bool PK = false>
-__device__ __forceinline__ void ipass_p4(uint32_t (&x)[64], const v4i (&M)[4], v4i comp, v4i tv, Rsrc tab,
+template <bool PK = false, bool QR = false>
+__device__ __forceinline__ void ipass_p4(uint32_t (&x)[64], const v4i (&M)[4], v4i comp, v4i comp2, v4i tv, Rsrc tab,
                                          uint32_t tvo, uint32_t tso, const Mc& m, uint32_t* lds, const Th& h) {
+  static_assert(!(QR && kFold4), "a folded pass keeps the Montgomery matrix");
   const uint32_t tsb = kFold4 ? tw_b<kTwB4>(tso) : tso;
 #pragma unroll
   for (int c = 0; c < 16; ++c) {
@@ -542,9 +608,9 @@
     const v4i tn = c + 1 < 16 ? bld(tab, tvo, tso + (uint32_t)(c + 1) * 1024u) : tv;
     v4i D[4];
     if constexpr (PK)
-      tile<true, false>(D, M, a, v4i{0, 0, 0, 0});
+      tile<true, false, QR>(D, M, a, v4i{0, 0, 0, 0});
     else
-      tile<true, true>(D, M, a, comp);
+      tile<true, true, QR>(D, M, a, comp, comp2);
     if constexpr (kFold4) {
       uint32_t o[4];
       twist4<false>(o, D, tv, tab, tvo, 0, tsb + (uint32_t)c * 1024u, m);
@@ -553,7 +619,7 @@
     } else {
 #pragma unroll
       for (int i = 0; i < 4; ++i) {
-        const int32_t r = recomb<false>(D[0][i], D[1][i], D[2][i], D[3][i], m);
+        const int32_t r = recomb_x<QR, false>(D[0][i], D[1][i], D[2][i], D[3][i], m);
         x[p3(c, i)] = (uint32_t)mont<true>(r, tv[i], m) ^ K32;
       }
     }
@@ -598,7 +664,7 @@
     tile_fence();
   }
 }
-template <int C0>
+template <int C0, bool QR = false>
 __device__ __forceinline__ void ipass_p2(uint32_t (&x)[64], const v4i (&M)[4], const Mc& m) {
   const v4i z = {0, 0, 0, 0};
 #pragma unroll
@@ -608,10 +674,10 @@
 #pragma unroll
     for (int i = 0; i < 4; ++i) b[i] = (int)x[q2(c, i)];
     v4i D[4];
-    tile<false, false>(D, M, b, z);
+    tile<false, false, QR>(D, M, b, z);
 #pragma unroll
     for (int i = 0; i < 4; ++i)
-      x[q2(c, i)] = (uint32_t)recomb<true>(D[0][i], D[1][i], D[2][i], D[3][i], m) ^ K32;
+      x[q2(c, i)] = (uint32_t)recomb_x<QR, true>(D[0][i], D[1][i], D[2][i], D[3][i], m) ^ K32;
     pin4(x[q2(c, 0)], x[q2(c, 1)], x[q2(c, 2)], x[q2(c, 3)]);
     tile_fence();
   }
@@ -684,6 +750,15 @@
   int64_t K = (int64_t)((uint64_t)K32 << 32), K0 = 0;
   int32_t one = 1, s16 = 65536;
   asm volatile("" : "+s"(one), "+s"(s16), "+s"(K), "+s"(K0));
+  if constexpr (kQrAny) {
+    int32_t mu = ((const int32_t*)((const v4i*)mf + (size_t)l * kLimb + kQConst))[0];
+    uint32_t nq = 0u - lc.q, kq = K32 - (kQrC << 24), kq0 = 0u - (kQrC << 24);
+    asm volatile("" : "+s"(mu), "+s"(nq), "+s"(kq), "+s"(kq0));
+    r.m.mu = mu;
+    r.m.nq = nq;
+    r.m.kq = kq;
+    r.m.kq0 = kq0;
+  }
   r.m.K = K;
   r.m.K0 = K0;
   r.m.one = one;
@@ -700,18 +775,20 @@
   return (uint32_t)(uintptr_t)lds + PBASE + h.w * PSTRIDE + h.lam() * 16u;
 }
 template <bool SYNC1, int F4 = S_F4, bool Q4 = false, bool SYNCX = false, int NPARK = 0, uint32_t PBASE = 0,
-          uint32_t PSTRIDE = 0, bool F3 = kFold3, class EPI = NoEpi>
+          uint32_t PSTRIDE = 0, bool F3 = kFold3, int QR = 0, class EPI = NoEpi>
 __device__ __forceinline__ void fwd(uint32_t (&x2)[64], Rsrc src, uint32_t* lds, const Th& h, const Tabs& T,
                                     const EPI& epi = EPI{}) {
   const Mc& m = T.m;
   const uint32_t lo = h.lam() * 16u;
   v4i M[4];
-  load_mat(M, T.tab, S_F1, lo);
-  const v4i comp = bld(T.tab, lo, (uint32_t)kCompF1 * 16u);
+  constexpr bool Q1 = (QR & 1) != 0, Q3 = (QR & 2) != 0, Q4P = (QR & kQrP4) != 0;
+  load_mat(M, T.tab, Q1 ? S_QF1 : S_F1, lo);
+  const v4i comp = bld(T.tab, lo, (uint32_t)(Q1 ? kQCompF1 : kCompF1) * 16u);
+  const v4i comp2 = Q1 ? bld(T.tab, lo, (uint32_t)(kQCompF1 + 64) * 16u) : comp;
   uint32_t x1[64];
   load_p1(x1, src, h);
   MF_STAMP(1);
-  pass_p1<0, true>(x1, M, comp, m);
+  pass_p1<0, true, Q1>(x1, M, comp, comp2, m);
   MF_STAMP(2);
   if constexpr (SYNC1) __syncthreads();
   uint32_t wb[4], rb[4];
@@ -719,7 +796,7 @@
   if constexpr (Q4) {
     p1_bases4(wb, h);
     x_write_p1q<0>(x1, lds, wb);
-    pass_p1<8, true>(x1, M, comp, m);
+    pass_p1<8, true, Q1>(x1, M, comp, comp2, m);
     __syncthreads();
     p2_bases4(rb, h);
     x_read_p2q<0>(x2, lds, rb);
@@ -746,7 +823,7 @@
   } else {
   p1_bases(wb, h);
   x_write_p1<0>(x1, lds, wb);
-  pass_p1<8, true>(x1, M, comp, m);
+  pass_p1<8, true, Q1>(x1, M, comp, comp2, m);
   MF_STAMP(3);
   __syncthreads();
   MF_STAMP(4);
@@ -778,21 +855,23 @@
     for (int i = 0; i < 4; ++i) x2[4 * c + i] = (uint32_t)v[i];
   }
   swap_p2p3(x2);
-  load_mat(M, T.tab, S_F3, lo);
-  pass_p3(x2, M, T.tab, lo, (uint32_t)(kTw4fR + h.w * 1024) * 16u, m);
+  load_mat(M, T.tab, Q3 ? S_QF3 : S_F3, lo);
+  pass_p3<Q3>(x2, M, T.tab, lo, (uint32_t)(kTw4fR + h.w * 1024) * 16u, m);
   MF_STAMP(9);
   load_mat(M, T.tab, F4, lo);
-  pass_p4(x2, M, m, epi);
+  pass_p4<Q4P>(x2, M, m, epi);
   MF_STAMP(10);
 }
 
-template <bool LOAD, bool PK = false>
+template <bool LOAD, bool PK = false, int QR = 0>
 __device__ __forceinline__ void inv_x(uint32_t (&x2)[64], Rsrc pr, uint32_t* lds, const Th& h, const Tabs& T) {
   const Mc& m = T.m;
   const uint32_t lo = h.lam() * 16u;
   v4i M[4];
-  load_mat(M, T.tab, S_I4, lo);
-  const v4i comp = bld(T.tab, lo, (uint32_t)kCompI4 * 16u);
+  constexpr bool Q2 = (QR & 1) != 0, Q4 = (QR & 2) != 0;
+  load_mat(M, T.tab, Q4 ? S_QI4 : S_I4, lo);
+  const v4i comp = bld(T.tab, lo, (uint32_t)(Q4 ? kQCompI4 : kCompI4) * 16u);
+  const v4i comp2 = Q4 && !PK ? bld(T.tab, lo, (uint32_t)(kQCompI4 + 64) * 16u) : comp;
   const uint32_t t4s = (uint32_t)(kTw4iR + h.w * 1024) * 16u;
   const v4i tv0 = bld(T.tab, lo, t4s);
   if constexpr (LOAD) {
@@ -805,18 +884,18 @@
   } else {
     __syncthreads();
   }
-  ipass_p4<PK>(x2, M, comp, tv0, T.tab, lo, t4s, m, lds, h);
+  ipass_p4<PK, Q4>(x2, M, comp, comp2, tv0, T.tab, lo, t4s, m, lds, h);
   load_mat(M, T.tab, S_I3, lo);
   ipass_p3(x2, M, T.tab, h.g() * 16u, (uint32_t)(kTw3iR + h.w * 64) * 16u, m, lds, h);
   swap_q3p2(x2);
-  load_mat(M, T.tab, S_I2 + h.w, lo);
+  load_mat(M, T.tab, (Q2 ? S_QI2 : S_I2) + h.w, lo);
   uint32_t wb[4], rb[4];
   uint32_t x1[64];
-  ipass_p2<0>(x2, M, m);
+  ipass_p2<0, Q2>(x2, M, m);
   __syncthreads();
   p2_bases(rb, h);
   x_write_p2<0>(x2, lds, rb);
-  ipass_p2<8>(x2, M, m);
+  ipass_p2<8, Q2>(x2, M, m);
   __syncthreads();
   p1_bases(wb, h);
   x_read_p1<0>(x1, lds, wb);
@@ -832,7 +911,7 @@
 }
 __device__ __forceinline__ void inv(Rsrc pr, uint32_t* lds, const Th& h, const Tabs& T) {
   uint32_t x2[64];
-  inv_x<true>(x2, pr, lds, h, T);
+  inv_x<true, false, kQrNtt>(x2, pr, lds, h, T);
 }
 
 }
@@ -852,7 +931,7 @@
   const Rsrc pr = rsrc(p, kN * 4u);
   if constexpr (!INV) {
     uint32_t x[64];
-    fwd<false, S_F4, false, false, 0, 0, 0, kFold3 && kFold3Fwd>(x, pr, lds, h, T, [&](int cc, const int32_t (&r)[4], uint32_t (&)[64]) {
+    fwd<false, S_F4, false, false, 0, 0, 0, kFold3 && kFold3Fwd, kQrNttFwd>(x, pr, lds, h, T, [&](int cc, const int32_t (&r)[4], uint32_t (&)[64]) {
       bst<kStreamAux>(v4i{(int)canon(r[0], T.m.q), (int)canon(r[1], T.m.q), (int)canon(r[2], T.m.q), (int)canon(r[3], T.m.q)}, pr,
           p4_lane(h), p4_soff(h, cc));
     });
@@ -909,13 +988,13 @@
   constexpr int NP = SX ? RNT_MF_TENSOR_PARK : 0;
   constexpr uint32_t PB = 128u * 1024u, PS = 2048u;
   constexpr int MEAS = RNT_MF_TENSOR_MEAS;
-  fwd<false, S_F4, false, SX, NP, PB, PS>(x, rsrc(c0 + io, kN * 4u), lds, h, T, [&](int cc, const int32_t (&r)[4], uint32_t (&)[64]) {
+  fwd<false, S_F4, false, SX, NP, PB, PS, kFold3, kQrTensor>(x, rsrc(c0 + io, kN * 4u), lds, h, T, [&](int cc, const int32_t (&r)[4], uint32_t (&)[64]) {
     if constexpr (MEAS != 3) bst(canon4(r), R1, pl, p4_soff(h, cc));
   });
-  fwd<!SX, S_F4, false, SX, NP, PB, PS>(x, rsrc(c1 + io, kN * 4u), lds, h, T, [&](int cc, const int32_t (&r)[4], uint32_t (&)[64]) {
+  fwd<!SX, S_F4, false, SX, NP, PB, PS, kFold3, kQrTensor>(x, rsrc(c1 + io, kN * 4u), lds, h, T, [&](int cc, const int32_t (&r)[4], uint32_t (&)[64]) {
     if constexpr (MEAS != 1) bst(canon4(r), RS, pl, p4_soff(h, cc));
   });
-  fwd<!SX, S_F4, false, SX, NP, PB, PS>(x, rsrc(c0p + io, kN * 4u), lds, h, T, [&](int cc, const int32_t (&r)[4], uint32_t (&)[64]) {
+  fwd<!SX, S_F4, false, SX, NP, PB, PS, kFold3, kQrTensor>(x, rsrc(c0p + io, kN * 4u), lds, h, T, [&](int cc, const int32_t (&r)[4], uint32_t (&)[64]) {
     const v4i a0 = MEAS == 3 ? canon4(r) : bld(R1, pl, p4_soff(h, cc));
     const v4i a1 = MEAS == 1 ? canon4(r) : bld(RS, pl, p4_soff(h, cc));
     const v4i b = canon4(r);
@@ -928,7 +1007,7 @@
     bst<kLastAux>(o0, R0, pl, p4_soff(h, cc));
     if constexpr (MEAS != 2) bst(t, R2, pl, p4_soff(h, cc));
   });
-  fwd<!SX, S_F4, false, RNT_MF_TENSOR_PARK4 && SX, RNT_MF_TENSOR_PARK4 ? NP : 0, PB, PS>(x, rsrc(c1p + io, kN * 4u), lds, h, T, [&](int cc, const int32_t (&r)[4], uint32_t (&xx)[64]) {
+  fwd<!SX, S_F4, false, RNT_MF_TENSOR_PARK4 && SX, RNT_MF_TENSOR_PARK4 ? NP : 0, PB, PS, kFold3, kQrTensor>(x, rsrc(c1p + io, kN * 4u), lds, h, T, [&](int cc, const int32_t (&r)[4], uint32_t (&xx)[64]) {
     const v4i b = canon4(r);
     const v4i a0 = MEAS == 3 ? b : bld<kLastAux>(R1, pl, p4_soff(h, cc));
     const v4i a1 = MEAS == 1 ? b : bld<kLastAux>(RS, pl, p4_soff(h, cc));
@@ -949,7 +1028,7 @@
       bst<kLastAux>(v4i{(int)xx[p3(cc, 0)], (int)xx[p3(cc, 1)], (int)xx[p3(cc, 2)], (int)xx[p3(cc, 3)]}, RH, pl,
                     p4_soff(h, cc));
   });
-  inv_x<false>(x, R2, lds, h, T);
+  inv_x<false, false, kQrTensor>(x, R2, lds, h, T);
 }
 
 #ifndef RNT_MF_MUL_Q4
@@ -996,13 +1075,15 @@
   uint32_t x[64];
   auto hat = [&](int t) -> v4i& { return ((v4i*)(lds + kMulLdsBase) + h.w * (kMulLdsTiles * 64) + h.lam())[t * 64]; };
   constexpr int NP = RNT_MF_MUL_Q4 ? RNT_MF_MUL_PARK : 0;
-  fwd<false, S_F4S, false, RNT_MF_MUL_Q4 != 0, NP, kMulLdsBase * 4, kMulLdsTiles * 1024>(x, rsrc(a + o, kN * 4u), lds, h, T, [&](int cc, const int32_t (&r)[4], uint32_t (&)[64]) {
+  constexpr int QM = kQrMul | ((kQrMul & 1) ? kQrP4 : 0);
+  constexpr int FA = (kQrMul & 1) ? S_F4 : S_F4S, FB = (kQrMul & 1) ? S_QF4 : S_F4;
+  fwd<false, FA, false, RNT_MF_MUL_Q4 != 0, NP, kMulLdsBase * 4, kMulLdsTiles * 1024, kFold3, QM>(x, rsrc(a + o, kN * 4u), lds, h, T, [&](int cc, const int32_t (&r)[4], uint32_t (&)[64]) {
     if (cc >= 16 - kMulLdsTiles)
       hat(cc - (16 - kMulLdsTiles)) = v4i{r[0], r[1], r[2], r[3]};
     else if (cc >= RNT_MF_MUL_MEAS_SKIP)
       bst<RNT_MF_SLOT_ST_AUX>(v4i{r[0], r[1], r[2], r[3]}, RS, p4_lane(h), p4_soff(h, cc));
   });
-  fwd<!(RNT_MF_MUL_Q4 && RNT_MF_MUL_NOSYNC1), S_F4, RNT_MF_MUL_Q4 != 0, (NP > 0), NP, 0, 4096>(x, rsrc(b + o, kN * 4u), lds, h, T, [&](int cc, const int32_t (&r)[4], uint32_t (&xx)[64]) {
+  fwd<!(RNT_MF_MUL_Q4 && RNT_MF_MUL_NOSYNC1), FB, RNT_MF_MUL_Q4 != 0, (NP > 0), NP, 0, 4096, kFold3, QM>(x, rsrc(b + o, kN * 4u), lds, h, T, [&](int cc, const int32_t (&r)[4], uint32_t (&xx)[64]) {
     const v4i ah = cc >= 16 - kMulLdsTiles ? hat(cc - (16 - kMulLdsTiles))
                    : cc < RNT_MF_MUL_MEAS_SKIP ? v4i{r[0], r[1], r[2], r[3]} : bld(RS, p4_lane(h), p4_soff(h, cc));
 #pragma unroll
@@ -1011,7 +1092,7 @@
     }
     pin4(xx[p3(cc, 0)], xx[p3(cc, 1)], xx[p3(cc, 2)], xx[p3(cc, 3)]);
   });
-  inv_x<false, true>(x, rsrc(c + o, kN * 4u), lds, h, T);
+  inv_x<false, true, kQrMul>(x, rsrc(c + o, kN * 4u), lds, h, T);
 }
 
 namespace {
@@ -1079,6 +1160,20 @@
         return -1;
       }
     }
+    if (kQrAny) {
+      const uint64_t Bq = (1ull << 28) + (1ull << 20) + (1ull << 15), c8 = (uint64_t)kQrC << 8, c24 = (uint64_t)kQrC << 24;
+      const uint64_t mu = (1ull << 48) / q, rho = (1ull << 48) % q;
+      const uint64_t neg = Bq + c24 + (((Bq - c8) * rho) >> 32) + 1;
+      const int64_t pos = (int64_t)(Bq + q + (((Bq + c8) * rho) >> 32) + 1) - (int64_t)c24;
+      const uint64_t rq = pos > (int64_t)neg ? (uint64_t)pos : neg, lim = 0x7F7F7F7Full;
+      const bool ok = mu <= 0x7FFFFFFFull && rq <= lim &&
+                      (host::u128)rq * q / ((host::u128)1 << 33) + q / 2 + 1 < lim &&
+                      (host::u128)rq * rq / ((host::u128)1 << 32) + q / 2 + 1 < lim;
+      if (!ok) {
+        *err = "MFMA tables: the quotient-estimate reduction's bound exceeds the packed digit range for this prime";
+        return -1;
+      }
+    }
     uint64_t M0[16][16];
     for (int k = 0; k < 16; ++k) {
       uint64_t v[16] = {};
@@ -1136,6 +1231,19 @@
     for (int k = 0; k < 16; ++k)
       for (int j = 0; j < 16; ++j) W[k][j] = mulmod(powmod(beta1i, (uint64_t)k, q), Fi[k][j], q);
     expand(W, q, R, false, 0, slot(S_I1));
+    if (kQrAny) {
+      expand(M0, q, 1, false, 0, slot(S_QF1));
+      expand(F, q, 1, true, 0, slot(S_QF3));
+      expand(F, q, 1, false, 1, slot(S_QF4));
+      expand(Fi, q, 1, true, 1, slot(S_QI4));
+      for (int U = 0; U < 16; ++U) {
+        const uint64_t bei = itw[128 + 8 * U];
+        for (int k = 0; k < 16; ++k)
+          for (int j = 0; j < 16; ++j) W[k][j] = mulmod(powmod(bei, (uint64_t)k, q), Fi[k][j], q);
+        expand(W, q, 1, false, 0, slot(S_QI2 + U));
+      }
+      lt[(size_t)kQConst * 4] = (int32_t)(uint32_t)((1ull << 48) / q);
+    }
     const uint64_t bias = mulmod(R, (1ull << 30) % q, q);
     {
       int32_t cf[16], ci[16];
@@ -1155,6 +1263,29 @@
           c1[lam * 4 + i] = cf[4 * i + (lam >> 4)];
           c4[lam * 4 + i] = ci[lam & 15];
         }
+      if (kQrAny) {
+        const uint64_t pb = (1ull << 30) % q;
+        int32_t* q1 = lt + (size_t)kQCompF1 * 4;
+        int32_t* q4 = lt + (size_t)kQCompI4 * 4;
+        auto split = [](int32_t v, int32_t* v0, int32_t* v2) {
+          *v2 = (v + 32768) >> 16;
+          *v0 = v - *v2 * 65536;
+        };
+        for (int j = 0; j < 16; ++j) {
+          uint64_t s0 = 0, s1 = 0;
+          for (int k = 0; k < 16; ++k) {
+            s0 = (s0 + M0[j][k]) % q;
+            s1 = (s1 + Fi[j][k]) % q;
+          }
+          cf[j] = centred(mulmod(pb, s0, q), q);
+          ci[j] = centred(mulmod(pb, s1, q), q);
+        }
+        for (int lam = 0; lam < 64; ++lam)
+          for (int i = 0; i < 4; ++i) {
+            split(cf[4 * i + (lam >> 4)], &q1[lam * 4 + i], &q1[(64 + lam) * 4 + i]);
+            split(ci[lam & 15], &q4[lam * 4 + i], &q4[(64 + lam) * 4 + i]);
+          }
+      }
     }
     const uint64_t s16 = (1ull << 16) % q;
     auto put = [&](int32_t* tab, bool fold, int dist, size_t idx, uint64_t tv) {
```

After: 167,600, median of 6. 1.01x the previous value.
